# ishika28/Beyond-Binary-Fake-User-Detection-A-Credibility-Aware-Graph-based-Recommender-System

Hardware: NVIDIA B200
Metric: edges/sec (3-layer cred-weighted LightGCN fwd+bwd) (higher is better)
Workload: dtype f32

## Files before the change

### beyond-binary-fake-user-detection-a-credibility-aware-graph-based-recommender-system_b200/_lib.py

```python
from __future__ import annotations

import ctypes as C
import os
import pathlib
import subprocess

import torch

PKG_DIR = pathlib.Path(__file__).resolve().parent
LIB_PATH = PKG_DIR / "libcredgcn.so"
CSRC_DIR = PKG_DIR / "csrc"

VARIANTS = {"cu": 0, "v2": 1, "da": 2}
ORDERS = {"jacobi": 0, "gs": 1}
PRECISIONS = {"fp32": 0, "bf16x3": 1, "bf16": 2}
OPTIONS = {"L2_TABLE_BYTES": 0, "SPARSE_FIRST_ADJOINT": 1, "PDL": 2, "P2P_ONESHOT_MAX": 3, "P2P_TIMING": 4,
           "P2P_TIMEOUT_MS": 5, "EVAL_DEBUG": 6, "HOT_ROWS": 7, "EVAL_GROUPS": 8,
           "TOPK_CHUNK_USERS": 9}
LONG_ROW = 256
CHUNK = 256


class CgxError(RuntimeError):
    pass


class CsrStruct(C.Structure):
    _fields_ = [
        ("n_rows", C.c_int32), ("n_cols", C.c_int32), ("nnz", C.c_int64),
        ("indptr", C.c_void_p), ("idx", C.c_void_p), ("val_fwd", C.c_void_p), ("val_bwd", C.c_void_p),
        ("perm", C.c_void_p), ("n_long", C.c_int32), ("n_chunks", C.c_int32),
        ("chunk_ptr", C.c_void_p), ("chunk_row", C.c_void_p),
        ("n_huge", C.c_int32), ("reserved_", C.c_int32), ("arrive", C.c_void_p), ("work", C.c_void_p),
        ("idx_hint", C.c_void_p),
    ]


_P = C.c_void_p
_CSR = C.POINTER(CsrStruct)
_SIGNATURES = {
    "cgx_last_error": (C.c_char_p, []),
    "cgx_version": (C.c_int, []),
    "cgx_launch_count": (C.c_uint64, []),
    "cgx_emb_dim_supported": (C.c_int, [C.c_int32]),
    "cgx_set_option": (C.c_int, [C.c_int, C.c_int64, C.POINTER(C.c_int64)]),
    "cgx_get_option": (C.c_int64, [C.c_int]),
    "cgx_hot_hints_workspace_bytes": (C.c_size_t, [C.c_int32]),
    "cgx_hot_hints": (C.c_int, [_P, C.c_int64, C.c_int32, _P, C.c_int32, _P, _P, C.c_size_t, _P]),
    "cgx_comm_status": (C.c_int, [_P, C.c_size_t, C.c_int, C.POINTER(C.c_uint32)]),
    "cgx_graph_build_workspace_bytes": (C.c_size_t, [C.c_int64, C.c_int32, C.c_int32]),
    "cgx_graph_build": (C.c_int, [_P, _P, C.c_int64, C.c_int32, C.c_int32, _P, C.c_int, _P, _P, _P, _P, _P, _P,
                                  _P, _P, _P, _P, _P, _P, _P, _P, _P, C.c_int, _P, C.c_size_t, _P]),
    "cgx_user_csr": (C.c_int, [_P, _P, C.c_int64, C.c_int32, C.c_int32, _P, _P, _P, C.c_size_t, _P]),
    "cgx_row_schedule_workspace_bytes": (C.c_size_t, [C.c_int32]),
    "cgx_row_schedule": (C.c_int, [_P, C.c_int32, _P, C.POINTER(C.c_int32), C.POINTER(C.c_int32),
                                   C.POINTER(C.c_int32), _P, C.c_size_t, _P]),
    "cgx_row_schedule_chunks": (C.c_int, [C.c_int32, C.c_int32, C.c_int32, _P, _P, _P, C.c_size_t, _P]),
    "cgx_row_schedule_work": (C.c_int, [_P, _P, C.c_int32, C.c_int32, C.c_int32, _P, _P, _P, _P]),
    "cgx_spmm_workspace_bytes": (C.c_size_t, [_CSR, C.c_int32]),
    "cgx_spmm": (C.c_int, [_CSR, C.c_int, C.c_int32, _P, _P, _P, _P, C.c_float, _P, C.c_size_t, _P]),
    "cgx_spmm_sparse_rows": (C.c_int, [_CSR, C.c_int, C.c_int32, _P, _P, _P, _P, _P, C.c_float, _P, C.c_size_t, _P]),
    "cgx_row_flags": (C.c_int, [_P, C.c_int64, C.c_int32, _P, _P]),
    "cgx_spmm_ex": (C.c_int, [_CSR, C.c_int, C.c_int32, _P, _P, _P, _P, _P, _P, C.c_float, _P, C.c_size_t, _P]),
    "cgx_spmm_set_l2_table_bytes": (C.c_int64, [C.c_int64]),
    "cgx_propagate_workspace_bytes": (C.c_size_t, [_CSR, _CSR, C.c_int32]),
    "cgx_propagate_workspace_bytes_for": (C.c_size_t, [_CSR, _CSR, C.c_int32, C.c_int]),
    "cgx_propagate_fwd": (C.c_int, [_CSR, _CSR, C.c_int, C.c_int32, C.c_int32, _P, _P, _P, _P, _P,
                                    C.c_size_t, _P]),
    "cgx_propagate_fwd_layers": (C.c_int, [_CSR, _CSR, C.c_int, C.c_int32, C.c_int32, _P, _P, _P, _P, C.c_int32,
                                           C.c_int32, _P, _P, _P, _P, C.c_size_t, _P]),
    "cgx_propagate_bwd": (C.c_int, [_CSR, _CSR, C.c_int, C.c_int32, C.c_int32, _P, _P, _P, _P, _P,
                                    C.c_size_t, _P]),
    "cgx_propagate_bwd_flagged": (C.c_int, [_CSR, _CSR, C.c_int, C.c_int32, C.c_int32, _P, _P, _P, _P, _P, _P, _P,
                                            C.c_size_t, _P]),
    "cgx_propagate_bwd_frontier": (C.c_int, [_CSR, _CSR, C.c_int, C.c_int32, C.c_int32, _P, _P, _P, _P, _P, _P,
                                             _P, _P, C.c_size_t, _P]),
    "cgx_batch_frontier": (C.c_int, [_CSR, _P, _P, _P, C.c_int64, _P, _P, _P]),
    "cgx_bpr_mark_rows": (C.c_int, [_P, C.c_int64, C.c_int32, _P, _P, _P]),
    "cgx_bpr_clear_rows": (C.c_int, [_P, C.c_int64, C.c_int32, C.c_int32, _P, _P, _P, _P, _P]),
    "cgx_bpr_workspace_bytes": (C.c_size_t, [C.c_int64, C.c_int32, C.c_int32]),
    "cgx_bpr_plan_workspace_bytes": (C.c_size_t, [C.c_int64]),
    "cgx_bpr_plan": (C.c_int, [_P, _P, _P, C.c_int64, C.c_int32, C.c_int32, _P, _P, C.c_size_t, _P]),
    "cgx_bpr_fwd_bwd": (C.c_int, [_P, _P, _P, C.c_int64, C.c_int64, _P, C.c_int32, C.c_int32, C.c_int32, _P, _P, _P,
                                  _P, _P,
                                  C.c_float, C.c_float, _P, _P, _P, _P, _P, _P, C.c_size_t, _P]),
    "cgx_bpr_apply_ego": (C.c_int, [_P, _P, C.c_int64, C.c_int32, C.c_int32, _P, _P, _P, _P, _P]),
    "cgx_sampler_build_workspace_bytes": (C.c_size_t, [C.c_int32]),
    "cgx_sampler_build": (C.c_int, [_P, C.c_int32, C.c_double, _P, _P, _P, _P, _P, _P, C.c_size_t, _P]),
    "cgx_sample_triples": (C.c_int, [_P, C.c_int64, _P, _P, C.c_int32, _P, _P, _P, _P, _P, C.c_float,
                                     C.c_int32, C.c_uint64, C.c_uint64, _P, _P, _P, _P]),
    "cgx_tick": (C.c_int, [_P, _P]),
    "cgx_adam_step": (C.c_int, [_P, _P, _P, _P, C.c_int64, _P, _P, _P, _P, C.c_int64, C.c_float, C.c_float,
                                C.c_float, C.c_float, _P, C.c_int64, _P]),
    "cgx_comm_alloc": (C.c_int, [C.c_size_t, C.POINTER(C.c_void_p)]),
    "cgx_comm_free": (C.c_int, [_P]),
    "cgx_comm_ipc_handle": (C.c_int, [_P, _P]),
    "cgx_comm_ipc_open": (C.c_int, [_P, C.POINTER(C.c_void_p)]),
    "cgx_comm_ipc_close": (C.c_int, [_P]),
    "cgx_comm_allreduce": (C.c_int, [C.c_int, C.c_int, C.POINTER(C.c_void_p), C.c_size_t, C.c_size_t, C.c_size_t,
                                     C.c_int64, _P, _P]),
    "cgx_comm_allgather": (C.c_int, [C.c_int, C.c_int, C.POINTER(C.c_void_p), _P, C.c_size_t, C.c_size_t, C.c_int64,
                                     _P, _P]),
    "cgx_comm_allreduce_nvls": (C.c_int, [C.c_int, C.c_int, C.POINTER(C.c_void_p), _P, C.c_size_t, C.c_size_t,
                                          C.c_size_t, C.c_int64, _P, _P]),
    "cgx_comm_timing": (C.c_int, [_P]),
    "cgx_spmm_set_push_peers": (C.c_int, [C.POINTER(C.c_void_p), C.c_int]),
    "cgx_spmm_push": (C.c_int, [_CSR, C.c_int, C.c_int32, _P, _P, C.c_size_t, C.c_int, C.c_int, C.c_int32, _P,
                                C.c_size_t, _P]),
    "cgx_comm_allreduce_pushed": (C.c_int, [C.c_int, C.c_int, C.POINTER(C.c_void_p), C.c_size_t, C.c_size_t,
                                            C.c_size_t, C.c_int64, C.c_int32, C.c_int32, _P, _P]),
    "cgx_eval_topk_workspace_bytes": (C.c_size_t, [C.c_int64, C.c_int32, C.c_int32, C.c_int32, C.c_int]),
    "cgx_eval_topk": (C.c_int, [_P, C.c_int64, _P, _P, C.c_int32, C.c_int32, _P, _P, C.c_int32, C.c_int, _P,
                                _P, _P, C.c_size_t, _P]),
    "cgx_score_candidates": (C.c_int, [_P, _P, C.c_int64, C.c_int32, C.c_int32, _P, _P, _P, _P]),
    "cgx_eval_candidates": (C.c_int, [_P, C.c_int64, _P, _P, _P, _P, C.c_int32, C.c_int32, C.c_uint64, _P, _P]),
    "cgx_rank_candidates": (C.c_int, [_P, _P, C.c_int64, C.c_int32, _P, _P]),
    "cgx_eval_topk_uses_tensor_cores": (C.c_int, [C.c_int32, C.c_int32, C.c_int]),
    "cgx_eval_metrics_workspace_bytes": (C.c_size_t, [C.c_int64, C.c_int32]),
    "cgx_eval_metrics": (C.c_int, [_P, C.c_int64, C.c_int32, _P, _P, _P, _P, C.c_int32, _P, C.c_int32, _P, C.c_int64,
                                   _P, _P, _P, _P, C.c_size_t, _P]),
    "cgx_eval_coverage": (C.c_int, [_P, C.c_int32, C.c_int32, _P, _P]),
}
EXPORTED = tuple(_SIGNATURES)

_lib = None


def build_library(verbose: bool = False) -> pathlib.Path:
    out = subprocess.run(["make", "-C", str(CSRC_DIR), "-j8"], capture_output=True, text=True)
    if verbose or out.returncode != 0:
        print(out.stdout[-4000:], out.stderr[-4000:])
    if out.returncode != 0:
        raise CgxError("building libcredgcn.so failed (see output above)")
    return LIB_PATH


def lib() -> C.CDLL:
    global _lib
    if _lib is None:
        if not LIB_PATH.exists():
            raise CgxError(
                f"{LIB_PATH} is missing: the sm_100a extension has not been built. Run "
                f"`python -c 'import __graft_entry__ as g; g.build()'` (or `make -C {CSRC_DIR}`). "
                "There is no CPU fallback.")
        handle = C.CDLL(str(LIB_PATH))
        for name, (res, args) in _SIGNATURES.items():
            fn = getattr(handle, name)
            fn.restype, fn.argtypes = res, args
        _lib = handle
        for name, key in OPTIONS.items():
            env = os.environ.get(f"CGX_OPT_{name}")
            if env is not None:
                handle.cgx_set_option(key, int(env), None)
    return _lib


def set_option(name: str, value: int) -> int:
    prev = C.c_int64(0)
    check(lib().cgx_set_option(OPTIONS[name], int(value), C.byref(prev)))
    return int(prev.value)


def get_option(name: str) -> int:
    return int(lib().cgx_get_option(OPTIONS[name]))


def check(status: int) -> None:
    if status != 0:
        raise CgxError(f"libcredgcn error {status}: {lib().cgx_last_error().decode()}")


def ptr(t: torch.Tensor | None):
    if t is None:
        return None
    if not t.is_cuda:
        raise CgxError("credgcn ops need CUDA tensors: there is no CPU fallback")
    if not t.is_contiguous():
        raise CgxError("credgcn ops need contiguous tensors")
    return C.c_void_p(t.data_ptr())


def stream_ptr(device=None):
    return C.c_void_p(torch.cuda.current_stream(device).cuda_stream)


def workspace(nbytes: int, device) -> torch.Tensor:
    return torch.empty(max(int(nbytes), 256), dtype=torch.uint8, device=device)
```

### beyond-binary-fake-user-detection-a-credibility-aware-graph-based-recommender-system_b200/csrc/spmm.cu

```cuda
#include "common.cuh"

namespace cgx {

constexpr int SP_THREADS = 256;

__device__ __forceinline__ void fma4(float4& a, float v, const float4& x) {
  a.x = fmaf(v, x.x, a.x);
  a.y = fmaf(v, x.y, a.y);
  a.z = fmaf(v, x.z, a.z);
  a.w = fmaf(v, x.w, a.w);
}
__device__ __forceinline__ float4 add4(const float4& a, const float4& b) {
  return make_float4(a.x + b.x, a.y + b.y, a.z + b.z, a.w + b.w);
}
__device__ __forceinline__ float4 scale4(const float4& a, float s) {
  return make_float4(a.x * s, a.y * s, a.z * s, a.w * s);
}

enum { POL_NORMAL = 0, POL_FIRST = 1, POL_LAST = 2 };
template <int POL>
__device__ __forceinline__ void ld256(const float4* p, float4& a, float4& b) {
  if (POL == POL_LAST) {
    asm volatile("ld.global.nc.L1::no_allocate.L2::evict_last.v8.f32 {%0,%1,%2,%3,%4,%5,%6,%7}, [%8];"
                 : "=f"(a.x), "=f"(a.y), "=f"(a.z), "=f"(a.w), "=f"(b.x), "=f"(b.y), "=f"(b.z), "=f"(b.w)
                 : "l"(p));
  } else if (POL == POL_FIRST) {
    asm volatile("ld.global.nc.L1::no_allocate.L2::evict_first.v8.f32 {%0,%1,%2,%3,%4,%5,%6,%7}, [%8];"
                 : "=f"(a.x), "=f"(a.y), "=f"(a.z), "=f"(a.w), "=f"(b.x), "=f"(b.y), "=f"(b.z), "=f"(b.w)
                 : "l"(p));
  } else {
    asm volatile("ld.global.nc.v8.f32 {%0,%1,%2,%3,%4,%5,%6,%7}, [%8];"
                 : "=f"(a.x), "=f"(a.y), "=f"(a.z), "=f"(a.w), "=f"(b.x), "=f"(b.y), "=f"(b.z), "=f"(b.w)
                 : "l"(p));
  }
}
template <int POL>
__device__ __forceinline__ void ld256_rw(const float4* p, float4& a, float4& b) {
  if (POL == POL_FIRST) {
    asm volatile("ld.global.L1::no_allocate.L2::evict_first.v8.f32 {%0,%1,%2,%3,%4,%5,%6,%7}, [%8];"
                 : "=f"(a.x), "=f"(a.y), "=f"(a.z), "=f"(a.w), "=f"(b.x), "=f"(b.y), "=f"(b.z), "=f"(b.w)
                 : "l"(p)
                 : "memory");
  } else {
    asm volatile("ld.global.v8.f32 {%0,%1,%2,%3,%4,%5,%6,%7}, [%8];"
                 : "=f"(a.x), "=f"(a.y), "=f"(a.z), "=f"(a.w), "=f"(b.x), "=f"(b.y), "=f"(b.z), "=f"(b.w)
                 : "l"(p)
                 : "memory");
  }
}
template <int POL>
__device__ __forceinline__ void st256(float4* p, const float4& a, const float4& b) {
  if (POL == POL_FIRST) {
    asm volatile("st.global.L2::evict_first.v8.f32 [%0], {%1,%2,%3,%4,%5,%6,%7,%8};" ::"l"(p), "f"(a.x), "f"(a.y),
                 "f"(a.z), "f"(a.w), "f"(b.x), "f"(b.y), "f"(b.z), "f"(b.w)
                 : "memory");
  } else {
    asm volatile("st.global.v8.f32 [%0], {%1,%2,%3,%4,%5,%6,%7,%8};" ::"l"(p), "f"(a.x), "f"(a.y), "f"(a.z), "f"(a.w),
                 "f"(b.x), "f"(b.y), "f"(b.z), "f"(b.w)
                 : "memory");
  }
}
template <bool STREAM>
__device__ __forceinline__ int32_t ld_idx(const int32_t* p) {
  if (!STREAM) return __ldg(p);
  int32_t v;
  asm volatile("ld.global.nc.L1::no_allocate.b32 %0, [%1];" : "=r"(v) : "l"(p));
  return v;
}
template <bool STREAM>
__device__ __forceinline__ float ld_val(const float* p) {
  if (!STREAM) return __ldg(p);
  float v;
  asm volatile("ld.global.nc.L1::no_allocate.f32 %0, [%1];" : "=f"(v) : "l"(p));
  return v;
}

template <int G>
__device__ __forceinline__ unsigned group_mask() {
  if (G == 32) return 0xffffffffu;
  const unsigned lane = threadIdx.x & 31;
  return ((1u << (G & 31)) - 1u) << (lane & ~(G - 1));
}

template <int G, int V, bool HOT>
__device__ __forceinline__ void ld_row(const float4* __restrict__ X, int32_t c, int lane, float4 (&x)[V]) {
  constexpr int ROW4 = G * V;
  if constexpr (V == 2) {
    if constexpr (HOT) {
      const float4* p = X + int64_t(c & 0x7fffffff) * ROW4 + 2 * lane;
      if (c < 0) ld256<POL_LAST>(p, x[0], x[1]);
      else ld256<POL_FIRST>(p, x[0], x[1]);
    } else {
      ld256<POL_NORMAL>(X + int64_t(c) * ROW4 + 2 * lane, x[0], x[1]);
    }
  } else {
#pragma unroll
    for (int v = 0; v < V; ++v) x[v] = __ldg(X + int64_t(c) * ROW4 + lane * V + v);
  }
}

template <int G, int V, int UNR, bool NZ, bool HOT>
__device__ __forceinline__ void gather_batches(const int32_t* __restrict__ idx, const float* __restrict__ val,
                                               int32_t len, const float4* __restrict__ X, int lane,
                                               unsigned mask, int32_t c_nxt, float w_nxt, float4 (&acc)[V],
                                               const uint8_t* __restrict__ nz) {
  idx += G + lane;
  val += G + lane;
  for (int32_t rem = len; rem > 0; rem -= G, idx += G, val += G) {
    const int32_t c = c_nxt;
    float w = w_nxt;
    if (NZ) {
      if (w != 0.f && __ldg(nz + c) == 0) w = 0.f;
    }
    if (G + lane < rem) {
      c_nxt = ld_idx<HOT>(idx);
      w_nxt = ld_val<HOT>(val);
    }
    const int cnt = rem < G ? rem : G;
    for (int j0 = 0; j0 < cnt; j0 += UNR) {
      float4 x[UNR][V];
      float ww[UNR];
#pragma unroll
      for (int t = 0; t < UNR; ++t) {
        const int j = j0 + t;
        const int src = (j < G) ? j : (G - 1);
        const int32_t cj = __shfl_sync(mask, c, src, G);
        ww[t] = __shfl_sync(mask, w, src, G);
        if (j < cnt && (!NZ || ww[t] != 0.f)) {
          ld_row<G, V, HOT>(X, cj, lane, x[t]);
        } else {
          ww[t] = 0.f;
#pragma unroll
          for (int v = 0; v < V; ++v) x[t][v] = make_float4(0.f, 0.f, 0.f, 0.f);
        }
      }
#pragma unroll
      for (int t = 0; t < UNR; ++t) {
#pragma unroll
        for (int v = 0; v < V; ++v) fma4(acc[v], ww[t], x[t][v]);
      }
    }
  }
}

__constant__ char* c_push_base[16];
struct SpmmPush {
  unsigned long long off;
  int32_t rows_per;
  int32_t rank;
};

template <int G, int V, bool STREAM>
__device__ __forceinline__ void epilogue(int64_t row, int lane, const float4 (&y)[V], float4* __restrict__ Y,
                                         const float4* ACC_IN, float4* ACC_OUT, float acc_scale,
                                         const uint8_t* __restrict__ acc_nz, const SpmmPush ps) {
  constexpr int ROW4 = G * V;
  constexpr int POL = STREAM ? POL_FIRST : POL_NORMAL;
  const int64_t o = row * ROW4 + lane * V;
  float4 a[V];
#pragma unroll
  for (int v = 0; v < V; ++v) a[v] = make_float4(0.f, 0.f, 0.f, 0.f);
  if (ACC_OUT != nullptr && ACC_IN != nullptr && (acc_nz == nullptr || __ldg(acc_nz + row) != 0)) {
    if constexpr (V == 2) ld256_rw<POL>(ACC_IN + o, a[0], a[1]);
    else {
#pragma unroll
      for (int v = 0; v < V; ++v) a[v] = ACC_IN[o + v];
    }
  }
  if (ps.rows_per > 0) {
    const int owner = int(row / ps.rows_per);
    float4* ypush = reinterpret_cast<float4*>(c_push_base[owner] + ps.off) +
                    (int64_t(ps.rank) * ps.rows_per + (row - int64_t(owner) * ps.rows_per)) * ROW4 + lane * V;
    if constexpr (V == 2) st256<POL_NORMAL>(ypush, y[0], y[1]);
    else {
#pragma unroll
      for (int v = 0; v < V; ++v) ypush[v] = y[v];
    }
  }
  if (Y != nullptr) {
    if constexpr (V == 2) st256<POL>(Y + o, y[0], y[1]);
    else {
#pragma unroll
      for (int v = 0; v < V; ++v) Y[o + v] = y[v];
    }
  }
  if (ACC_OUT != nullptr) {
#pragma unroll
    for (int v = 0; v < V; ++v) a[v] = scale4(add4(a[v], y[v]), acc_scale);
    if constexpr (V == 2) st256<POL>(ACC_OUT + o, a[0], a[1]);
    else {
#pragma unroll
      for (int v = 0; v < V; ++v) ACC_OUT[o + v] = a[v];
    }
  }
}

struct SpmmSched {
  const int32_t* perm;
  const int32_t* chunk_ptr;
  int32_t* arrive;
  int32_t n_chunks, n_huge;
};

template <int G, int V, int UNR, int MINB, bool NZ, bool PUSH, bool HOT>
__global__ void __launch_bounds__(SP_THREADS, MINB) k_spmm(const int32_t* __restrict__ idx,
                                                           const float* __restrict__ val, int64_t n_items,
                                                           SpmmSched sc, const float4* __restrict__ X,
                                                           float4* __restrict__ Y, const float4* ACC_IN,
                                                           float4* ACC_OUT, float acc_scale, float4* partial,
                                                           const uint8_t* __restrict__ nz,
                                                           const uint8_t* __restrict__ acc_nz,
                                                           const uint8_t* __restrict__ out_rows,
                                                           const int4* __restrict__ work, const SpmmPush ps_in) {
  const SpmmPush ps = PUSH ? ps_in : SpmmPush{0ull, 0, 0};
  constexpr int ROW4 = G * V;
  asm volatile("griddepcontrol.launch_dependents;");
  const int lane = threadIdx.x & (G - 1);
  const uint32_t item = (blockIdx.x * uint32_t(SP_THREADS) + threadIdx.x) / G;
  const unsigned mask = group_mask<G>();
  float4 acc[V];
#pragma unroll
  for (int v = 0; v < V; ++v) acc[v] = make_float4(0.f, 0.f, 0.f, 0.f);
  if (item >= n_items) return;
  const int4 wd = __ldg(work + item);
  const int64_t begin = (int64_t(wd.y) << 32) | uint32_t(wd.x);
  idx += begin;
  val += begin;
  int32_t cf = 0;
  float wf = 0.f;
  if (lane < wd.z) {
    cf = ld_idx<HOT>(idx + lane);
    wf = ld_val<HOT>(val + lane);
  }
  asm volatile("griddepcontrol.wait;" ::: "memory");
  if (NZ && !PUSH && out_rows != nullptr &&
      __ldg(out_rows + (item >= sc.n_chunks ? wd.w : __ldg(sc.perm + wd.w))) == 0)
    return;
  gather_batches<G, V, UNR, NZ, HOT>(idx, val, wd.z, X, lane, mask, cf, wf, acc, nz);
  if (item >= sc.n_chunks) {
    epilogue<G, V, HOT>(wd.w, lane, acc, Y, ACC_IN, ACC_OUT, acc_scale, acc_nz, ps);
    return;
  }
  const int32_t k = wd.w;
#pragma unroll
  for (int v = 0; v < V; ++v) __stcg(partial + int64_t(item) * ROW4 + lane * V + v, acc[v]);
  if (k < sc.n_huge) return;
  const int32_t c0 = __ldg(sc.chunk_ptr + k), c1 = __ldg(sc.chunk_ptr + k + 1);
  __threadfence();
  __syncwarp(mask);
  int prev = 0;
  if (lane == 0) prev = atomicAdd(sc.arrive + k, 1);
  prev = __shfl_sync(mask, prev, 0, G);
  if (prev != c1 - c0 - 1) return;
  __threadfence();
#pragma unroll
  for (int v = 0; v < V; ++v) acc[v] = make_float4(0.f, 0.f, 0.f, 0.f);
  for (int c = c0; c < c1; ++c) {
#pragma unroll
    for (int v = 0; v < V; ++v) acc[v] = add4(acc[v], __ldcg(partial + int64_t(c) * ROW4 + lane * V + v));
  }
  epilogue<G, V, HOT>(int64_t(__ldg(sc.perm + k)), lane, acc, Y, ACC_IN, ACC_OUT, acc_scale, acc_nz, ps);
  if (lane == 0) sc.arrive[k] = 0;
}

template <int G, int V>
__global__ void __launch_bounds__(SP_THREADS) k_spmm_finish(SpmmSched sc, const float4* __restrict__ partial,
                                                            float4* __restrict__ Y, const float4* ACC_IN,
                                                            float4* ACC_OUT, float acc_scale,
                                                            const uint8_t* __restrict__ acc_nz,
                                                            const uint8_t* __restrict__ out_rows, const SpmmPush ps) {
  constexpr int GROUPS = SP_THREADS / G;
  constexpr int ROW4 = G * V;
  __shared__ float4 red[GROUPS][ROW4];
  const int k = blockIdx.x;
  if (out_rows != nullptr && __ldg(out_rows + __ldg(sc.perm + k)) == 0) return;
  const int lane = threadIdx.x & (G - 1), grp = threadIdx.x / G;
  const int c0 = __ldg(sc.chunk_ptr + k), c1 = __ldg(sc.chunk_ptr + k + 1);
  float4 acc[V];
#pragma unroll
  for (int v = 0; v < V; ++v) acc[v] = make_float4(0.f, 0.f, 0.f, 0.f);
  for (int c = c0 + grp; c < c1; c += GROUPS) {
#pragma unroll
    for (int v = 0; v < V; ++v) acc[v] = add4(acc[v], __ldg(partial + int64_t(c) * ROW4 + lane * V + v));
  }
#pragma unroll
  for (int v = 0; v < V; ++v) red[grp][lane * V + v] = acc[v];
  __syncthreads();
  if (grp == 0) {
#pragma unroll
    for (int v = 0; v < V; ++v) {
      float4 s = red[0][lane * V + v];
      for (int g = 1; g < GROUPS; ++g) s = add4(s, red[g][lane * V + v]);
      acc[v] = s;
    }
    epilogue<G, V, false>(int64_t(__ldg(sc.perm + k)), lane, acc, Y, ACC_IN, ACC_OUT, acc_scale, acc_nz, ps);
  }
}

__global__ void k_scale(const float4* __restrict__ in, float4* __restrict__ out, int64_t n4, float s) {
  int64_t p = int64_t(blockIdx.x) * blockDim.x + threadIdx.x;
  if (p < n4) out[p] = scale4(in[p], s);
}

__global__ void k_row_flags(const uint4* __restrict__ X, int64_t n4, int32_t row4, uint8_t* __restrict__ flags) {
  const int64_t p = int64_t(blockIdx.x) * blockDim.x + threadIdx.x;
  if (p >= n4) return;
  const uint4 v = X[p];
  if ((v.x | v.y | v.z | v.w) & 0x7fffffffu) flags[p / row4] = 1;
}

static int row_flags(const float* X, int64_t n_rows, int32_t d, uint8_t* flags, cudaStream_t stream) {
  CGX_CUDA(cudaMemsetAsync(flags, 0, size_t(n_rows), stream));
  const int64_t n4 = n_rows * d / 4;
  if (n4 == 0) return CGX_OK;
  k_row_flags<<<(unsigned)ceil_div(n4, 256), 256, 0, stream>>>(reinterpret_cast<const uint4*>(X), n4, d / 4, flags);
  CGX_LAUNCH_CHECK();
  return CGX_OK;
}

template <int G, int V, int UNR, int MINB, bool NZ, bool PUSH, bool HOT>
static int launch_spmm(const cgx_csr* m, const float* val, const float* X, float* Y, const float* ACC_IN,
                       float* ACC_OUT, float acc_scale, void* workspace, size_t workspace_bytes,
                       cudaStream_t stream, const uint8_t* nz, const uint8_t* acc_nz, const uint8_t* out_rows,
                       const SpmmPush ps) {
  constexpr int GROUPS = SP_THREADS / G;
  float4* partial = nullptr;
  if (m->n_long > 0) {
    size_t need = size_t(m->n_chunks) * G * V * sizeof(float4);
    CGX_REQUIRE(workspace != nullptr && workspace_bytes >= need, CGX_ERR_WORKSPACE,
                "spmm: workspace too small for %d long-row chunks", m->n_chunks);
    partial = static_cast<float4*>(workspace);
  }
  SpmmSched sc{m->perm, m->chunk_ptr, m->arrive, m->n_chunks, m->n_huge};
  const int64_t items = int64_t(m->n_chunks) + (m->n_rows - m->n_long);
  cudaLaunchConfig_t cfg = {};
  cfg.gridDim = dim3((unsigned)ceil_div(items, GROUPS));
  cfg.blockDim = dim3(SP_THREADS);
  cfg.dynamicSmemBytes = 0;
  cfg.stream = stream;
  cudaLaunchAttribute attr[1];
  attr[0].id = cudaLaunchAttributeProgrammaticStreamSerialization;
  attr[0].val.programmaticStreamSerializationAllowed = option(CGX_OPT_PDL) != 0 ? 1 : 0;
  cfg.attrs = attr;
  cfg.numAttrs = 1;
  CGX_CUDA(cudaLaunchKernelEx(&cfg, k_spmm<G, V, UNR, MINB, NZ, PUSH, HOT>, HOT ? m->idx_hint : m->idx, val, items, sc,
                              reinterpret_cast<const float4*>(X), reinterpret_cast<float4*>(Y),
                              reinterpret_cast<const float4*>(ACC_IN), reinterpret_cast<float4*>(ACC_OUT), acc_scale,
                              partial, nz, acc_nz, out_rows, static_cast<const int4*>(m->work), ps));
  CGX_LAUNCH_CHECK();
  if (m->n_huge > 0) {
    k_spmm_finish<G, V><<<(unsigned)m->n_huge, SP_THREADS, 0, stream>>>(
        sc, partial, reinterpret_cast<float4*>(Y), reinterpret_cast<const float4*>(ACC_IN),
        reinterpret_cast<float4*>(ACC_OUT), acc_scale, acc_nz, out_rows, ps);
    CGX_LAUNCH_CHECK();
  }
  return CGX_OK;
}

#define CGX_SPMM_ARGS m, val, X, Y, ACC_IN, ACC_OUT, acc_scale, ws, ws_bytes, stream, nz, acc_nz, out_rows, ps

template <int G, int V, int UNR>
static int spmm_flavour(const cgx_csr* m, const float* val, const float* X, float* Y, const float* ACC_IN,
                        float* ACC_OUT, float acc_scale, void* ws, size_t ws_bytes, cudaStream_t stream,
                        const uint8_t* nz, const uint8_t* acc_nz, const uint8_t* out_rows, const SpmmPush ps,
                        bool hot) {
  const bool push = ps.rows_per > 0;
  if constexpr (V == 2) {
    if (hot && nz == nullptr) {
      if (push) return launch_spmm<G, V, UNR, 4, false, true, true>(CGX_SPMM_ARGS);
      return launch_spmm<G, V, UNR, 4, false, false, true>(CGX_SPMM_ARGS);
    }
  }
  if (push) {
    if (nz) return launch_spmm<G, V, UNR, 4, true, true, false>(CGX_SPMM_ARGS);
    return launch_spmm<G, V, UNR, 4, false, true, false>(CGX_SPMM_ARGS);
  }
  if (nz) return launch_spmm<G, V, UNR, 4, true, false, false>(CGX_SPMM_ARGS);
  return launch_spmm<G, V, UNR, 4, false, false, false>(CGX_SPMM_ARGS);
}

#define CGX_FLAVOUR_ARGS m, val, X, Y, ACC_IN, ACC_OUT, acc_scale, ws, ws_bytes, stream, nz, acc_nz, out_rows, ps, hot

static int spmm_dispatch(const cgx_csr* m, int use_bwd, int32_t d, const float* X, float* Y, const float* ACC_IN,
                         float* ACC_OUT, float acc_scale, void* ws, size_t ws_bytes, cudaStream_t stream,
                         const uint8_t* nz = nullptr, const SpmmPush ps = SpmmPush{0ull, 0, 0},
                         const uint8_t* acc_nz = nullptr, const uint8_t* out_rows = nullptr) {
  CGX_REQUIRE(m && m->perm && m->work && (m->nnz == 0 || (m->idx && m->val_fwd && m->val_bwd)) && X, CGX_ERR_ARG,
              "spmm: NULL pointer (cgx_csr needs idx, both value arrays and the cgx_row_schedule* outputs)");
  CGX_REQUIRE(m->n_long == 0 || (m->chunk_ptr && m->arrive), CGX_ERR_ARG, "spmm: chunk tables missing");
  CGX_REQUIRE(Y || ACC_OUT || ps.rows_per > 0, CGX_ERR_ARG, "spmm: no output requested");
  CGX_REQUIRE(out_rows == nullptr || (nz != nullptr && ps.rows_per == 0), CGX_ERR_ARG,
              "spmm: an output-row mask needs gather flags and no push mode");
  const float* val = use_bwd ? m->val_bwd : m->val_fwd;
  if (m->n_rows == 0) return CGX_OK;
  const bool beyond_l2 = int64_t(m->n_cols) * int64_t(d) * 4 > option(CGX_OPT_L2_TABLE_BYTES);
  const bool hot = beyond_l2 && m->idx_hint != nullptr && option(CGX_OPT_HOT_ROWS) != 0;
  switch (d) {
    case 16: return spmm_flavour<4, 1, 4>(CGX_FLAVOUR_ARGS);
    case 32: return spmm_flavour<8, 1, 8>(CGX_FLAVOUR_ARGS);
    case 64:
      if (beyond_l2) return spmm_flavour<8, 2, 4>(CGX_FLAVOUR_ARGS);
      return spmm_flavour<16, 1, 8>(CGX_FLAVOUR_ARGS);
    case 128:
      if (beyond_l2) return spmm_flavour<16, 2, 4>(CGX_FLAVOUR_ARGS);
      return spmm_flavour<32, 1, 8>(CGX_FLAVOUR_ARGS);
    case 256: return spmm_flavour<32, 2, 4>(CGX_FLAVOUR_ARGS);
    default:
      set_error("spmm: emb_dim %d unsupported (16, 32, 64, 128, 256)", d);
      return CGX_ERR_UNSUPPORTED;
  }
}

__global__ void k_hot_flags(const int32_t* __restrict__ col_by_degree, int32_t n_hot, uint8_t* __restrict__ hot) {
  const int32_t k = blockIdx.x * blockDim.x + threadIdx.x;
  if (k < n_hot) hot[__ldg(col_by_degree + k)] = 1;
}
__global__ void k_hot_hint(const int32_t* __restrict__ idx, int64_t nnz, const uint8_t* __restrict__ hot,
                           int32_t* __restrict__ out) {
  const int64_t p = int64_t(blockIdx.x) * blockDim.x + threadIdx.x;
  if (p >= nnz) return;
  const int32_t c = idx[p];
  out[p] = __ldg(hot + c) ? (c | int32_t(0x80000000u)) : c;
}

static size_t spmm_ws(const cgx_csr* m, int32_t d) { return align_up(size_t(m ? m->n_chunks : 0) * d * 4); }

}

using namespace cgx;

extern "C" size_t cgx_spmm_workspace_bytes(const cgx_csr* m, int32_t d) { return spmm_ws(m, d); }

extern "C" int cgx_spmm(const cgx_csr* m, int use_bwd_values, int32_t d, const float* X, float* Y,
                        const float* ACC_IN, float* ACC_OUT, float acc_scale, void* workspace,
                        size_t workspace_bytes, void* stream) {
  return spmm_dispatch(m, use_bwd_values, d, X, Y, ACC_IN, ACC_OUT, acc_scale, workspace, workspace_bytes,
                       static_cast<cudaStream_t>(stream));
}

extern "C" int cgx_spmm_sparse_rows(const cgx_csr* m, int use_bwd_values, int32_t d, const float* X,
                                    const uint8_t* x_row_nonzero, float* Y, const float* ACC_IN, float* ACC_OUT,
                                    float acc_scale, void* workspace, size_t workspace_bytes, void* stream) {
  CGX_REQUIRE(x_row_nonzero != nullptr, CGX_ERR_ARG, "spmm_sparse_rows: NULL flags");
  return spmm_dispatch(m, use_bwd_values, d, X, Y, ACC_IN, ACC_OUT, acc_scale, workspace, workspace_bytes,
                       static_cast<cudaStream_t>(stream), x_row_nonzero);
}

extern "C" int cgx_spmm_ex(const cgx_csr* m, int use_bwd_values, int32_t d, const float* X, const uint8_t* x_row_nonzero,
                           float* Y, const float* ACC_IN, const uint8_t* acc_row_nonzero, float* ACC_OUT,
                           float acc_scale, void* workspace, size_t workspace_bytes, void* stream) {
  return spmm_dispatch(m, use_bwd_values, d, X, Y, ACC_IN, ACC_OUT, acc_scale, workspace, workspace_bytes,
                       static_cast<cudaStream_t>(stream), x_row_nonzero, SpmmPush{0ull, 0, 0}, acc_row_nonzero);
}

extern "C" int64_t cgx_spmm_set_l2_table_bytes(int64_t bytes) {
  int64_t old = 0;
  cgx_set_option(CGX_OPT_L2_TABLE_BYTES, bytes, &old);
  return old;
}

extern "C" size_t cgx_hot_hints_workspace_bytes(int32_t n_cols) { return align_up(size_t(n_cols > 0 ? n_cols : 0)) + 256; }

extern "C" int cgx_hot_hints(const int32_t* idx, int64_t nnz, int32_t n_cols, const int32_t* col_by_degree,
                             int32_t n_hot, int32_t* idx_hint, void* workspace, size_t workspace_bytes,
                             void* stream_) {
  cudaStream_t stream = static_cast<cudaStream_t>(stream_);
  CGX_REQUIRE(nnz >= 0 && n_cols > 0 && col_by_degree && idx_hint && (nnz == 0 || idx) && n_hot >= 0 &&
                  n_hot <= n_cols,
              CGX_ERR_ARG, "hot_hints: bad argument");
  CGX_REQUIRE(workspace != nullptr && workspace_bytes >= cgx_hot_hints_workspace_bytes(n_cols), CGX_ERR_WORKSPACE,
              "hot_hints: workspace too small");
  uint8_t* hot = static_cast<uint8_t*>(workspace);
  CGX_CUDA(cudaMemsetAsync(hot, 0, size_t(n_cols), stream));
  if (n_hot > 0) {
    k_hot_flags<<<(unsigned)ceil_div(n_hot, 256), 256, 0, stream>>>(col_by_degree, n_hot, hot);
    CGX_LAUNCH_CHECK();
  }
  if (nnz > 0) {
    k_hot_hint<<<(unsigned)ceil_div(nnz, 256), 256, 0, stream>>>(idx, nnz, hot, idx_hint);
    CGX_LAUNCH_CHECK();
  }
  return CGX_OK;
}

extern "C" int cgx_spmm_set_push_peers(void* const* peer_bases, int world) {
  CGX_REQUIRE(peer_bases != nullptr && world >= 1 && world <= 16, CGX_ERR_ARG, "spmm_set_push_peers: bad argument");
  char* h[16] = {nullptr};
  for (int p = 0; p < world; ++p) h[p] = static_cast<char*>(peer_bases[p]);
  CGX_CUDA(cudaMemcpyToSymbol(c_push_base, h, sizeof(h)));
  return CGX_OK;
}

extern "C" int cgx_spmm_push(const cgx_csr* m, int use_bwd_values, int32_t d, const float* X,
                             const uint8_t* x_row_nonzero, size_t stage_off, int rank, int world, int32_t rows_per,
                             void* workspace, size_t workspace_bytes, void* stream) {
  CGX_REQUIRE(m != nullptr && world >= 1 && world <= 16 && rank >= 0 && rank < world && rows_per > 0 &&
                  int64_t(rows_per) * world >= m->n_rows && stage_off % 16 == 0,
              CGX_ERR_ARG, "spmm_push: bad rank / world / rows_per");
  const SpmmPush ps{(unsigned long long)stage_off, rows_per, rank};
  return spmm_dispatch(m, use_bwd_values, d, X, nullptr, nullptr, nullptr, 1.0f, workspace, workspace_bytes,
                       static_cast<cudaStream_t>(stream), x_row_nonzero, ps);
}

extern "C" int cgx_row_flags(const float* X, int64_t n_rows, int32_t d, uint8_t* flags, void* stream) {
  CGX_REQUIRE(X && flags && n_rows >= 0 && d > 0 && d % 4 == 0, CGX_ERR_ARG, "row_flags: bad argument");
  return row_flags(X, n_rows, d, flags, static_cast<cudaStream_t>(stream));
}

__device__ __forceinline__ int64_t clamp_row(int64_t x, int64_t n) { return (x < 0 || x >= n) ? 0 : x; }
__global__ void k_batch_frontier(const int64_t* __restrict__ indptr, const int32_t* __restrict__ idx,
                                 const int64_t* __restrict__ users, const int64_t* __restrict__ pos,
                                 const int64_t* __restrict__ neg, int64_t B, int32_t U, int32_t I,
                                 uint8_t* __restrict__ flags, uint8_t* __restrict__ flags_u) {
  const int64_t t = (int64_t(blockIdx.x) * blockDim.x + threadIdx.x) / 32;
  const int lane = threadIdx.x & 31;
  if (t >= B) return;
  const int64_t u = clamp_row(users[t], U);
  if (lane == 0) {
    flags[clamp_row(pos[t], I)] = 1;
    flags[clamp_row(neg[t], I)] = 1;
    if (flags_u != nullptr) flags_u[u] = 1;
  }
  const int64_t end = indptr[u + 1];
  for (int64_t j = indptr[u] + lane; j < end; j += 32) flags[idx[j]] = 1;
}

extern "C" int cgx_batch_frontier(const cgx_csr* by_user, const int64_t* users, const int64_t* pos,
                                  const int64_t* neg, int64_t B, uint8_t* flags_i, uint8_t* flags_u,
                                  void* stream_) {
  cudaStream_t stream = static_cast<cudaStream_t>(stream_);
  CGX_REQUIRE(by_user && by_user->indptr && (by_user->nnz == 0 || by_user->idx) && users && pos && neg && flags_i,
              CGX_ERR_ARG, "batch_frontier: NULL pointer");
  CGX_REQUIRE(B > 0 && B < (int64_t(1) << 29) && by_user->n_rows > 0 && by_user->n_cols > 0, CGX_ERR_ARG,
              "batch_frontier: bad batch size %lld or empty graph", (long long)B);
  CGX_CUDA(cudaMemsetAsync(flags_i, 0, size_t(by_user->n_cols), stream));
  if (flags_u != nullptr) CGX_CUDA(cudaMemsetAsync(flags_u, 0, size_t(by_user->n_rows), stream));
  k_batch_frontier<<<(unsigned)ceil_div(B * 32, 256), 256, 0, stream>>>(
      by_user->indptr, by_user->idx, users, pos, neg, B, by_user->n_rows, by_user->n_cols, flags_i, flags_u);
  CGX_LAUNCH_CHECK();
  return CGX_OK;
}

static size_t propagate_ws(const cgx_csr* by_user, const cgx_csr* by_item, int32_t d, int n_buf) {
  if (!by_user || !by_item) return 0;
  size_t long_ws = spmm_ws(by_user, d) > spmm_ws(by_item, d) ? spmm_ws(by_user, d) : spmm_ws(by_item, d);
  return n_buf * (align_up(size_t(by_user->n_rows) * d * 4) + align_up(size_t(by_item->n_rows) * d * 4)) + long_ws +
         align_up(size_t(by_user->n_rows)) + align_up(size_t(by_item->n_rows)) + 256;
}

extern "C" size_t cgx_propagate_workspace_bytes(const cgx_csr* by_user, const cgx_csr* by_item, int32_t d) {
  return propagate_ws(by_user, by_item, d, 2);
}

extern "C" size_t cgx_propagate_workspace_bytes_for(const cgx_csr* by_user, const cgx_csr* by_item, int32_t d,
                                                    int order) {
  return propagate_ws(by_user, by_item, d, order == CGX_ORDER_GS ? 1 : 2);
}

extern "C" int cgx_propagate_fwd(const cgx_csr* by_user, const cgx_csr* by_item, int order, int32_t K, int32_t d,
                                 const float* e0_u, const float* e0_i, float* out_u, float* out_i,
                                 void* workspace, size_t workspace_bytes, void* stream) {
  return cgx_propagate_fwd_layers(by_user, by_item, order, K, d, e0_u, e0_i, out_u, out_i, 0, K, nullptr, nullptr,
                                  nullptr, workspace, workspace_bytes, stream);
}

extern "C" int cgx_propagate_fwd_layers(const cgx_csr* by_user, const cgx_csr* by_item, int order, int32_t K,
                                        int32_t d, const float* e0_u, const float* e0_i, float* out_u, float* out_i,
                                        int32_t layer_begin, int32_t layer_end, const uint8_t* rows_u,
                                        const uint8_t* rows_i, const uint8_t* all_rows, void* workspace,
                                        size_t workspace_bytes, void* stream_) {
  cudaStream_t stream = static_cast<cudaStream_t>(stream_);
  CGX_REQUIRE(by_user && by_item && e0_u && e0_i && out_u && out_i, CGX_ERR_ARG, "propagate_fwd: NULL pointer");
  CGX_REQUIRE(K >= 1, CGX_ERR_ARG, "propagate_fwd: num_layers must be >= 1");
  CGX_REQUIRE(0 <= layer_begin && layer_begin <= layer_end && layer_end <= K, CGX_ERR_ARG,
              "propagate_fwd: layers [%d, %d) outside [0, %d)", layer_begin, layer_end, K);
  CGX_REQUIRE((rows_u == nullptr && rows_i == nullptr) || all_rows != nullptr, CGX_ERR_ARG,
              "propagate_fwd: output-row masks need all_rows");
  CGX_REQUIRE(order == CGX_ORDER_JACOBI || order == CGX_ORDER_GS, CGX_ERR_ARG, "propagate_fwd: bad order");
  CGX_REQUIRE(by_user->n_rows == by_item->n_cols && by_user->n_cols == by_item->n_rows, CGX_ERR_ARG,
              "propagate_fwd: operator shapes disagree");
  CGX_REQUIRE(workspace_bytes >= cgx_propagate_workspace_bytes_for(by_user, by_item, d, order), CGX_ERR_WORKSPACE,
              "propagate_fwd: workspace too small");
  const int64_t U = by_user->n_rows, I = by_item->n_rows;
  Arena ws(workspace, workspace_bytes);
  const bool one = order == CGX_ORDER_GS;
  float* ub[2];
  float* ib[2];
  ub[0] = ws.take<float>(U * d);
  ub[1] = one ? ub[0] : ws.take<float>(U * d);
  ib[0] = ws.take<float>(I * d);
  ib[1] = one ? ib[0] : ws.take<float>(I * d);
  size_t lws = spmm_ws(by_user, d) > spmm_ws(by_item, d) ? spmm_ws(by_user, d) : spmm_ws(by_item, d);
  void* lw = ws.take<char>(lws);
  CGX_REQUIRE(ws.ok, CGX_ERR_WORKSPACE, "propagate_fwd: workspace too small");
  const float s = 1.0f / float(K + 1);
  const SpmmPush nops{0ull, 0, 0};
  for (int k = layer_begin; k < layer_end; ++k) {
    const bool first = k == 0, last = k == K - 1;
    const float* cu = first ? e0_u : ub[(k - 1) & 1];
    const float* ci = first ? e0_i : ib[(k - 1) & 1];
    float* nu = ub[k & 1];
    float* ni = ib[k & 1];
    const float sc = last ? s : 1.0f;
    const uint8_t* mu = last ? rows_u : nullptr;
    const uint8_t* mi = last ? rows_i : nullptr;
    const bool need_ni = !last || order == CGX_ORDER_GS;
    CGX_TRY(spmm_dispatch(by_item, 0, d, cu, need_ni ? ni : nullptr, first ? e0_i : out_i, out_i, sc, lw, lws,
                          stream, mi ? all_rows : nullptr, nops, nullptr, mi));
    const float* src = order == CGX_ORDER_JACOBI ? ci : ni;
    CGX_TRY(spmm_dispatch(by_user, 0, d, src, last ? nullptr : nu, first ? e0_u : out_u, out_u, sc, lw, lws,
                          stream, mu ? all_rows : nullptr, nops, nullptr, mu));
  }
  return CGX_OK;
}

__global__ void k_scale_rows(const float4* __restrict__ in, const uint8_t* __restrict__ nz, float4* __restrict__ out,
                             int64_t n_rows, int32_t row4, float s) {
  const int64_t r = (int64_t(blockIdx.x) * blockDim.x + threadIdx.x) / 32;
  if (r >= n_rows || __ldg(nz + r) == 0) return;
  for (int p = threadIdx.x & 31; p < row4; p += 32) out[r * row4 + p] = scale4(in[r * row4 + p], s);
}

extern "C" int cgx_propagate_bwd(const cgx_csr* by_user, const cgx_csr* by_item, int order, int32_t K, int32_t d,
                                 const float* g_u, const float* g_i, float* d_e0_u, float* d_e0_i,
                                 void* workspace, size_t workspace_bytes, void* stream_) {
  return cgx_propagate_bwd_flagged(by_user, by_item, order, K, d, g_u, g_i, nullptr, nullptr, d_e0_u, d_e0_i, workspace,
                                   workspace_bytes, stream_);
}

extern "C" int cgx_propagate_bwd_flagged(const cgx_csr* by_user, const cgx_csr* by_item, int order, int32_t K,
                                         int32_t d, const float* g_u, const float* g_i, const uint8_t* g_u_rows,
                                         const uint8_t* g_i_rows, float* d_e0_u, float* d_e0_i, void* workspace,
                                         size_t workspace_bytes, void* stream_) {
  return cgx_propagate_bwd_frontier(by_user, by_item, order, K, d, g_u, g_i, g_u_rows, g_i_rows, nullptr, d_e0_u,
                                    d_e0_i, workspace, workspace_bytes, stream_);
}

extern "C" int cgx_propagate_bwd_frontier(const cgx_csr* by_user, const cgx_csr* by_item, int order, int32_t K,
                                          int32_t d, const float* g_u, const float* g_i, const uint8_t* g_u_rows,
                                          const uint8_t* g_i_rows, const uint8_t* front_i, float* d_e0_u,
                                          float* d_e0_i, void* workspace, size_t workspace_bytes, void* stream_) {
  cudaStream_t stream = static_cast<cudaStream_t>(stream_);
  CGX_REQUIRE((g_u_rows == nullptr) == (g_i_rows == nullptr), CGX_ERR_ARG,
              "propagate_bwd_flagged: pass both row-flag arrays or neither");
  CGX_REQUIRE(by_user && by_item && g_u && g_i && d_e0_u && d_e0_i, CGX_ERR_ARG, "propagate_bwd: NULL pointer");
  CGX_REQUIRE(K >= 1, CGX_ERR_ARG, "propagate_bwd: num_layers must be >= 1");
  CGX_REQUIRE(order == CGX_ORDER_JACOBI || order == CGX_ORDER_GS, CGX_ERR_ARG, "propagate_bwd: bad order");
  CGX_REQUIRE(workspace_bytes >= cgx_propagate_workspace_bytes_for(by_user, by_item, d, order), CGX_ERR_WORKSPACE,
              "propagate_bwd: workspace too small");
  const int64_t U = by_user->n_rows, I = by_item->n_rows;
  Arena ws(workspace, workspace_bytes);
  const bool one = order == CGX_ORDER_GS;
  float* ub[2];
  float* ib[2];
  ub[0] = ws.take<float>(U * d);
  ub[1] = one ? ub[0] : ws.take<float>(U * d);
  ib[0] = ws.take<float>(I * d);
  ib[1] = one ? ib[0] : ws.take<float>(I * d);
  size_t lws = spmm_ws(by_user, d) > spmm_ws(by_item, d) ? spmm_ws(by_user, d) : spmm_ws(by_item, d);
  void* lw = ws.take<char>(lws);
  CGX_REQUIRE(ws.ok, CGX_ERR_WORKSPACE, "propagate_bwd: workspace too small");
  const float s = 1.0f / float(K + 1);
  const bool given = g_u_rows != nullptr;
  const bool sparse = given || option(CGX_OPT_SPARSE_FIRST_ADJOINT) != 0;
  uint8_t* nz_u = given ? const_cast<uint8_t*>(g_u_rows) : ws.take<uint8_t>(U);
  uint8_t* nz_i = given ? const_cast<uint8_t*>(g_i_rows) : ws.take<uint8_t>(I);
  CGX_REQUIRE(ws.ok, CGX_ERR_WORKSPACE, "propagate_bwd: workspace too small");
  const uint8_t* front = sparse ? front_i : nullptr;
  if (order == CGX_ORDER_JACOBI) {
    const float* bu = g_u;
    const float* bi = g_i;
    if (sparse && !given) {
      CGX_TRY(row_flags(g_u, U, d, nz_u, stream));
      CGX_TRY(row_flags(g_i, I, d, nz_i, stream));
    }
    for (int k = 0; k < K; ++k) {
      const bool last = k == K - 1;
      float* nu = last ? d_e0_u : ub[k & 1];
      float* ni = last ? d_e0_i : ib[k & 1];
      const float sc = last ? s : 1.0f;
      const bool sp = sparse && k == 0;
      const SpmmPush nops{0ull, 0, 0};
      const uint8_t* bi_nz = sp ? nz_i : (k == 1 ? front : nullptr);
      CGX_TRY(spmm_dispatch(by_user, 1, d, bi, nullptr, g_u, nu, sc, lw, lws, stream, bi_nz, nops,
                            sparse ? nz_u : nullptr));
      CGX_TRY(spmm_dispatch(by_item, 1, d, bu, nullptr, g_i, ni, sc, lw, lws, stream, sp ? nz_u : nullptr, nops,
                            sparse ? nz_i : nullptr, k == 0 && !last ? front : nullptr));
      bu = nu;
      bi = ni;
    }
  } else {
    const float* bu = g_u;
    if (sparse && !given) {
      CGX_TRY(row_flags(g_u, U, d, nz_u, stream));
      CGX_TRY(row_flags(g_i, I, d, nz_i, stream));
    }
    const SpmmPush nops{0ull, 0, 0};
    for (int k = 0; k < K; ++k) {
      const bool last = k == K - 1;
      float* ni = ib[0];
      float* nu = last ? d_e0_u : ub[k & 1];
      const uint8_t* f0 = k == 0 ? front : nullptr;
      CGX_TRY(spmm_dispatch(by_item, 1, d, bu, nullptr, g_i, ni, 1.0f, lw, lws, stream,
                            sparse && k == 0 ? nz_u : nullptr, nops, sparse ? nz_i : nullptr, f0));
      CGX_TRY(spmm_dispatch(by_user, 1, d, ni, nullptr, g_u, nu, last ? s : 1.0f, lw, lws, stream, f0, nops,
                            sparse ? nz_u : nullptr));
      bu = nu;
    }
    const int64_t n4 = I * d / 4;
    if (given) {
      CGX_CUDA(cudaMemsetAsync(d_e0_i, 0, size_t(I) * d * 4, stream));
      if (I > 0) {
        k_scale_rows<<<(unsigned)ceil_div(I * 32, 256), 256, 0, stream>>>(
            reinterpret_cast<const float4*>(g_i), nz_i, reinterpret_cast<float4*>(d_e0_i), I, d / 4, s);
        CGX_LAUNCH_CHECK();
      }
    } else {
      k_scale<<<(unsigned)ceil_div(n4, 256), 256, 0, stream>>>(reinterpret_cast<const float4*>(g_i),
                                                               reinterpret_cast<float4*>(d_e0_i), n4, s);
      CGX_LAUNCH_CHECK();
    }
  }
  return CGX_OK;
}
```

### beyond-binary-fake-user-detection-a-credibility-aware-graph-based-recommender-system_b200/model.py

```python
from __future__ import annotations

import torch

from . import _lib
from ._lib import check, lib, ptr, stream_ptr, workspace
from .graph import CredGraph, graph_of


def _f32c(t: torch.Tensor) -> torch.Tensor:
    if t.dtype != torch.float32:
        raise _lib.CgxError(f"credgcn kernels are fp32, got {t.dtype}")
    return t.contiguous()


def _i64c(t, device) -> torch.Tensor:
    return torch.as_tensor(t, device=device).to(torch.int64).contiguous()


def propagate_forward(graph: CredGraph, e0_u, e0_i, num_layers: int, order: str):
    e0_u, e0_i = _f32c(e0_u), _f32c(e0_i)
    d = e0_u.shape[1]
    out_u, out_i = torch.empty_like(e0_u), torch.empty_like(e0_i)
    ws = graph.propagate_workspace(d, order)
    with torch.cuda.device(graph.device):
        check(lib().cgx_propagate_fwd(graph.by_user.ref(), graph.by_item.ref(), _lib.ORDERS[order], num_layers, d,
                                      ptr(e0_u), ptr(e0_i), ptr(out_u), ptr(out_i), ptr(ws), ws.numel(),
                                      stream_ptr(graph.device)))
    return out_u, out_i


def propagate_backward(graph: CredGraph, g_u, g_i, num_layers: int, order: str):
    g_u, g_i = _f32c(g_u), _f32c(g_i)
    d = g_u.shape[1]
    d_u, d_i = torch.empty_like(g_u), torch.empty_like(g_i)
    ws = graph.propagate_workspace(d, order)
    with torch.cuda.device(graph.device):
        check(lib().cgx_propagate_bwd(graph.by_user.ref(), graph.by_item.ref(), _lib.ORDERS[order], num_layers, d,
                                      ptr(g_u), ptr(g_i), ptr(d_u), ptr(d_i), ptr(ws), ws.numel(),
                                      stream_ptr(graph.device)))
    return d_u, d_i


def spmm(csr, x, use_bwd_values=False):
    x = _f32c(x)
    d = x.shape[1]
    y = torch.empty(csr.n_rows, d, dtype=torch.float32, device=x.device)
    ws = workspace(lib().cgx_spmm_workspace_bytes(csr.ref(), d), x.device)
    with torch.cuda.device(x.device):
        check(lib().cgx_spmm(csr.ref(), int(use_bwd_values), d, ptr(x), ptr(y), None, None, 1.0, ptr(ws),
                             ws.numel(), stream_ptr(x.device)))
    return y


def row_flags(x):
    x = _f32c(x)
    flags = torch.empty(x.shape[0], dtype=torch.uint8, device=x.device)
    with torch.cuda.device(x.device):
        check(lib().cgx_row_flags(ptr(x), x.shape[0], x.shape[1], ptr(flags), stream_ptr(x.device)))
    return flags


def spmm_sparse_rows(csr, x, flags=None, use_bwd_values=False):
    x = _f32c(x)
    flags = row_flags(x) if flags is None else flags
    d = x.shape[1]
    y = torch.empty(csr.n_rows, d, dtype=torch.float32, device=x.device)
    ws = workspace(lib().cgx_spmm_workspace_bytes(csr.ref(), d), x.device)
    with torch.cuda.device(x.device):
        check(lib().cgx_spmm_sparse_rows(csr.ref(), int(use_bwd_values), d, ptr(x), ptr(flags), ptr(y), None, None,
                                         1.0, ptr(ws), ws.numel(), stream_ptr(x.device)))
    return y


def bpr_plan(graph: CredGraph, users, pos, neg, plan=None):
    dev = graph.device
    users, pos, neg = _i64c(users, dev), _i64c(pos, dev), _i64c(neg, dev)
    B = users.numel()
    if plan is None:
        plan = torch.empty(3 * B, dtype=torch.int64, device=dev)
    ws = workspace(lib().cgx_bpr_plan_workspace_bytes(B), dev)
    with torch.cuda.device(dev):
        check(lib().cgx_bpr_plan(ptr(users), ptr(pos), ptr(neg), B, graph.num_users, graph.num_items, ptr(plan),
                                 ptr(ws), ws.numel(), stream_ptr(dev)))
    return plan


def batch_frontier(graph: CredGraph, users, pos, neg, flags=None, flags_u=None):
    dev = graph.device
    users, pos, neg = _i64c(users, dev), _i64c(pos, dev), _i64c(neg, dev)
    if flags is None:
        flags = torch.empty(graph.num_items, dtype=torch.uint8, device=dev)
    with torch.cuda.device(dev):
        check(lib().cgx_batch_frontier(graph.by_user.ref(), ptr(users), ptr(pos), ptr(neg), users.numel(), ptr(flags),
                                       ptr(flags_u), stream_ptr(dev)))
    return flags


def bpr_fused(graph: CredGraph, f_u, f_i, e0_u, e0_i, users, pos, neg, reg_weight, fair_weight=0.0, pop=None,
              g_u=None, g_i=None, plan=None, bufs=None, batch_total=0):
    dev = f_u.device
    f_u, f_i, e0_u, e0_i = _f32c(f_u), _f32c(f_i), _f32c(e0_u), _f32c(e0_i)
    users, pos, neg = _i64c(users, dev), _i64c(pos, dev), _i64c(neg, dev)
    B, d = users.numel(), f_u.shape[1]
    if plan is None:
        plan = bpr_plan(graph, users, pos, neg)
    if g_u is None:
        g_u = torch.zeros_like(f_u)
    if g_i is None:
        g_i = torch.zeros_like(f_i)
    if bufs is None:
        bufs = bpr_buffers(graph, B, dev)
    loss, ego_rows, ego_coef, ws = bufs
    pop_t = None if pop is None else _f32c(torch.as_tensor(pop, device=dev))
    with torch.cuda.device(dev):
        check(lib().cgx_bpr_fwd_bwd(ptr(users), ptr(pos), ptr(neg), B, int(batch_total), ptr(plan), graph.num_users,
                                    graph.num_items,
                                    d, ptr(f_u), ptr(f_i), ptr(e0_u), ptr(e0_i), ptr(pop_t), float(reg_weight),
                                    float(fair_weight), ptr(loss), ptr(g_u), ptr(g_i), ptr(ego_rows),
                                    ptr(ego_coef), ptr(ws), ws.numel(), stream_ptr(dev)))
    return loss, g_u, g_i, ego_rows, ego_coef


def bpr_buffers(graph: CredGraph, B: int, dev):
    return (torch.empty(1, dtype=torch.float32, device=dev), torch.empty(3 * B, dtype=torch.int32, device=dev),
            torch.empty(3 * B, dtype=torch.float32, device=dev),
            workspace(lib().cgx_bpr_workspace_bytes(B, graph.num_users, graph.num_items), dev))


def apply_ego(graph: CredGraph, ego_rows, ego_coef, e0_u, e0_i, d_e0_u, d_e0_i):
    with torch.cuda.device(e0_u.device):
        check(lib().cgx_bpr_apply_ego(ptr(ego_rows), ptr(ego_coef), ego_rows.numel(), graph.num_users,
                                      e0_u.shape[1], ptr(_f32c(e0_u)), ptr(_f32c(e0_i)), ptr(d_e0_u), ptr(d_e0_i),
                                      stream_ptr(e0_u.device)))


class _Propagate(torch.autograd.Function):

    @staticmethod
    def forward(ctx, e0_u, e0_i, graph, num_layers, order):
        ctx.graph, ctx.num_layers, ctx.order = graph, num_layers, order
        return propagate_forward(graph, e0_u.detach(), e0_i.detach(), num_layers, order)

    @staticmethod
    def backward(ctx, g_u, g_i):
        d_u, d_i = propagate_backward(ctx.graph, g_u, g_i, ctx.num_layers, ctx.order)
        return d_u, d_i, None, None, None


class _SpMM(torch.autograd.Function):

    @staticmethod
    def forward(ctx, x, graph, which):
        ctx.graph, ctx.which = graph, which
        return spmm(graph.by_user if which == "A" else graph.by_item, x.detach(), False)

    @staticmethod
    def backward(ctx, gy):
        csr = ctx.graph.by_item if ctx.which == "A" else ctx.graph.by_user
        return spmm(csr, gy, True), None, None


class _BprLoss(torch.autograd.Function):
    @staticmethod
    def forward(ctx, f_u, f_i, e0_u, e0_i, graph, users, pos, neg, reg_weight, fair_weight, pop):
        loss, g_u, g_i, ego_rows, ego_coef = bpr_fused(graph, f_u.detach(), f_i.detach(), e0_u.detach(),
                                                        e0_i.detach(), users, pos, neg, reg_weight, fair_weight, pop)
        ctx.graph = graph
        ctx.save_for_backward(g_u, g_i, ego_rows, ego_coef, e0_u.detach(), e0_i.detach())
        return loss.reshape(())

    @staticmethod
    def backward(ctx, g):
        g_u, g_i, ego_rows, ego_coef, e0_u, e0_i = ctx.saved_tensors
        d_e0_u, d_e0_i = torch.zeros_like(e0_u), torch.zeros_like(e0_i)
        apply_ego(ctx.graph, ego_rows, ego_coef, e0_u, e0_i, d_e0_u, d_e0_i)
        return g_u * g, g_i * g, d_e0_u * g, d_e0_i * g, None, None, None, None, None, None, None


def fused_bpr_loss(graph, f_u, f_i, e0_u, e0_i, users, pos, neg, reg_weight, fair_weight=0.0, pop=None):
    return _BprLoss.apply(f_u, f_i, e0_u, e0_i, graph, users, pos, neg, reg_weight, fair_weight, pop)


class _Base(torch.nn.Module):
    ORDER = "gs"

    def __init__(self, num_users, num_items, emb_dim, num_layers, M_ui, M_iu):
        super().__init__()
        self.num_users, self.num_items, self.num_layers = num_users, num_items, num_layers
        self.M_ui, self.M_iu = M_ui, M_iu
        self.graph = graph_of(M_ui, M_iu)
        if (self.graph.num_users, self.graph.num_items) != (num_users, num_items):
            raise ValueError("operator shapes do not match num_users / num_items")
        if not lib().cgx_emb_dim_supported(emb_dim):
            raise _lib.CgxError(f"emb_dim={emb_dim} unsupported: use 16, 32, 64, 128 or 256")
        self.user_emb = torch.nn.Embedding(num_users, emb_dim)
        self.item_emb = torch.nn.Embedding(num_items, emb_dim)
        torch.nn.init.xavier_uniform_(self.user_emb.weight)
        torch.nn.init.xavier_uniform_(self.item_emb.weight)

    def ego_tables(self):
        eu, ei = self.user_emb.weight, self.item_emb.weight
        eu.grad, ei.grad = torch.empty_like(eu), torch.empty_like(ei)
        return eu.data, ei.data, eu.grad, ei.grad

    def _final(self):
        return _Propagate.apply(self.user_emb.weight, self.item_emb.weight, self.graph, self.num_layers, self.ORDER)

    def _layers(self):
        u, i = self.user_emb.weight, self.item_emb.weight
        us, is_ = [u], [i]
        for _ in range(self.num_layers):
            i_new = _SpMM.apply(u, self.graph, "C")
            u_new = _SpMM.apply(i if self.ORDER == "jacobi" else i_new, self.graph, "A")
            u, i = u_new, i_new
            us.append(u)
            is_.append(i)
        return us, is_


class CredLightGCN(_Base):
    ORDER = "jacobi"

    def propagate_all_layers(self):
        return self._layers()

    def final_embeddings(self):
        return self._final()

    def score(self, users, items, e_u, e_i):
        return (e_u[users] * e_i[items]).sum(dim=1)

    def l2_reg(self, users, pos_items, neg_items):
        eu, ep, en = self.user_emb.weight[users], self.item_emb.weight[pos_items], self.item_emb.weight[neg_items]
        return (eu.norm(2, dim=1).pow(2) + ep.norm(2, dim=1).pow(2) + en.norm(2, dim=1).pow(2)).mean()

    def fused_loss(self, users, pos_items, neg_items, e_u, e_i, lambda_reg, lambda_fair=0.0, pop=None):
        return fused_bpr_loss(self.graph, e_u, e_i, self.user_emb.weight, self.item_emb.weight, users, pos_items,
                              neg_items, lambda_reg, lambda_fair, pop)


class LightGCN(_Base):
    ORDER = "gs"

    def propagate(self):
        return self._final()

    def get_user_item_emb(self):
        return self.propagate()

    def bpr_loss(self, users, pos_items, neg_items, user_emb, item_emb, reg_weight: float):
        return fused_bpr_loss(self.graph, user_emb, item_emb, self.user_emb.weight, self.item_emb.weight, users,
                              pos_items, neg_items, reg_weight)


class RawLightGCN(torch.nn.Module):
    ORDER = "jacobi"

    def __init__(self, num_users, num_items, emb_dim, num_layers, norm_adj):
        super().__init__()
        from .graph import NormAdj
        if not isinstance(norm_adj, NormAdj):
            raise TypeError("expected the handle returned by credgcn.graph.build_norm_adj")
        self.num_users, self.num_items, self.num_layers = num_users, num_items, num_layers
        self.num_nodes = num_users + num_items
        self.norm_adj, self.graph = norm_adj, norm_adj.graph
        if not lib().cgx_emb_dim_supported(emb_dim):
            raise _lib.CgxError(f"emb_dim={emb_dim} unsupported: use 16, 32, 64, 128 or 256")
        self.emb = torch.nn.Embedding(self.num_nodes, emb_dim)
        torch.nn.init.xavier_uniform_(self.emb.weight)

    def ego_tables(self):
        w, U = self.emb.weight, self.num_users
        w.grad = torch.empty_like(w)
        return w.data[:U], w.data[U:], w.grad[:U], w.grad[U:]

    def propagate(self):
        w = self.emb.weight
        fu, fi = _Propagate.apply(w[: self.num_users], w[self.num_users:], self.graph, self.num_layers, self.ORDER)
        return torch.cat([fu, fi], dim=0)

    def get_user_item_emb(self):
        x = self.propagate()
        return x[: self.num_users], x[self.num_users:]

    def bpr_loss(self, users, pos_items, neg_items, user_emb, item_emb, reg_weight: float):
        w = self.emb.weight
        return fused_bpr_loss(self.graph, user_emb, item_emb, w[: self.num_users], w[self.num_users:], users,
                              pos_items, neg_items, reg_weight)


class FusedAdam:

    def __init__(self, user_weight: torch.Tensor, item_weight: torch.Tensor, lr=1e-3, betas=(0.9, 0.999), eps=1e-8,
                 grads=None):
        self.params = (user_weight, item_weight)
        self.grads = grads
        self.lr, self.betas, self.eps = float(lr), (float(betas[0]), float(betas[1])), float(eps)
        self.m = [torch.zeros_like(p) for p in self.params]
        self.v = [torch.zeros_like(p) for p in self.params]
        self.step_dev = torch.zeros(1, dtype=torch.int64, device=user_weight.device)

    def _grads(self):
        return self.grads if self.grads is not None else tuple(p.grad for p in self.params)

    def zero_grad(self, set_to_none: bool = False):
        for g in self._grads():
            if g is not None:
                g.zero_()

    @torch.no_grad()
    def step(self):
        pu, pi = self.params
        gu, gi = self._grads()
        dev = pu.device
        with torch.cuda.device(dev):
            st = stream_ptr(dev)
            check(lib().cgx_tick(ptr(self.step_dev), st))
            check(lib().cgx_adam_step(ptr(pu.data), ptr(_f32c(gu)), ptr(self.m[0]), ptr(self.v[0]), pu.numel(),
                                      ptr(pi.data), ptr(_f32c(gi)), ptr(self.m[1]), ptr(self.v[1]), pi.numel(),
                                      self.lr, self.betas[0], self.betas[1], self.eps, ptr(self.step_dev), 0, st))

    def state_dict(self):
        return {"step": int(self.step_dev.item()), "exp_avg": self.m, "exp_avg_sq": self.v, "lr": self.lr,
                "betas": self.betas, "eps": self.eps}


class TrainStep:

    DEFER_HEADROOM = 2 << 30

    def __init__(self, model: _Base | RawLightGCN, lr=1e-3, reg_weight=1e-4, fair_weight=0.0, pop=None, optimizer=None,
                 sampler=None):
        self.model, self.graph = model, model.graph
        self.reg, self.fair = float(reg_weight), float(fair_weight)
        self._eu, self._ei, self._gu, self._gi = model.ego_tables()
        eu, ei = self._eu, self._ei
        dev = eu.device
        self.pop = None if pop is None else torch.as_tensor(pop, dtype=torch.float32, device=dev).contiguous()
        self._f_u, self._f_i = torch.empty_like(eu), torch.empty_like(ei)
        self.g_u, self.g_i = torch.zeros_like(eu), torch.zeros_like(ei)
        self.nz_u = torch.zeros(eu.shape[0], dtype=torch.uint8, device=dev)
        self.nz_i = torch.zeros(ei.shape[0], dtype=torch.uint8, device=dev)
        self.front_i = torch.zeros(ei.shape[0], dtype=torch.uint8, device=dev)
        self.batch_u = torch.zeros(eu.shape[0], dtype=torch.uint8, device=dev)
        self.opt = optimizer or FusedAdam(eu, ei, lr=lr, grads=(self._gu, self._gi))
        self.sampler = sampler
        self.phase_events = None
        self.side = torch.cuda.Stream(device=dev)
        self.tick = torch.zeros(1, dtype=torch.int64, device=dev)
        self._bufs = {}
        self._graph = None
        self._defer_final = None
        self._fws = self._all_rows = None
        self._pending = False
        self._final_error = None

    @property
    def f_u(self) -> torch.Tensor:
        self._complete_final()
        return self._f_u

    @property
    def f_i(self) -> torch.Tensor:
        self._complete_final()
        return self._f_i

    def _defers_final(self, d, order, beyond_l2):
        if self.model.num_layers < 2 or not beyond_l2:
            return False
        g = self.graph
        need = lib().cgx_propagate_workspace_bytes_for(g.by_user.ref(), g.by_item.ref(), d, order)
        free, _ = torch.cuda.mem_get_info(g.device)
        return free >= need + self.DEFER_HEADROOM

    @torch.no_grad()
    def _complete_final(self):
        if self._final_error is not None:
            raise self._final_error
        if not self._pending:
            return
        m, g = self.model, self.graph
        eu, ei = self._eu, self._ei
        d, K, order = eu.shape[1], m.num_layers, _lib.ORDERS[m.ORDER]
        dev = eu.device
        with torch.cuda.device(dev):
            rest_u = torch.eq(self.batch_u, 0).view(torch.uint8)
            rest_i = torch.eq(self.front_i, 0).view(torch.uint8)
            try:
                check(lib().cgx_propagate_fwd_layers(g.by_user.ref(), g.by_item.ref(), order, K, d, ptr(eu), ptr(ei),
                                                     ptr(self._f_u), ptr(self._f_i), K - 1, K, ptr(rest_u),
                                                     ptr(rest_i), ptr(self._all_rows), ptr(self._fws),
                                                     self._fws.numel(), stream_ptr(dev)))
            except _lib.CgxError as e:
                self._final_error = e
                raise
        self._pending = False

    def _mark(self, marks):
        if self.phase_events is not None:
            ev = torch.cuda.Event(enable_timing=True)
            ev.record(torch.cuda.current_stream(self.graph.device))
            marks.append(ev)

    def _batch_bufs(self, B, dev):
        if B not in self._bufs:
            self._bufs[B] = (torch.empty(3 * B, dtype=torch.int64, device=dev), bpr_buffers(self.graph, B, dev))
        return self._bufs[B]

    @torch.no_grad()
    def forward_backward(self, users, pos, neg):
        m, g = self.model, self.graph
        eu, ei = self._eu, self._ei
        d, K, order = eu.shape[1], m.num_layers, _lib.ORDERS[m.ORDER]
        ws = g.propagate_workspace(d, order)
        dev = eu.device
        users, pos, neg = _i64c(users, dev), _i64c(pos, dev), _i64c(neg, dev)
        plan, bufs = self._batch_bufs(users.numel(), dev)
        beyond_l2 = g.num_items * d * 4 > _lib.get_option("L2_TABLE_BYTES")
        if self._defer_final is None:
            self._defer_final = self._defers_final(d, order, beyond_l2)
        defer = bool(self._defer_final) and K >= 2
        if defer and self._fws is None:
            self._fws = workspace(lib().cgx_propagate_workspace_bytes_for(g.by_user.ref(), g.by_item.ref(), d, order),
                                  dev)
            self._all_rows = torch.ones(max(g.num_users, g.num_items), dtype=torch.uint8, device=dev)
        front = self.front_i if beyond_l2 or defer else None
        marks = []
        self._pending, self._final_error = False, None
        with torch.cuda.device(dev):
            main = torch.cuda.current_stream(dev)
            self._mark(marks)
            self.side.wait_stream(main)
            with torch.cuda.stream(self.side):
                bpr_plan(g, users, pos, neg, plan)
                if front is not None:
                    batch_frontier(g, users, pos, neg, front, self.batch_u if defer else None)
            st = stream_ptr(dev)
            if defer:
                fws = self._fws
                check(lib().cgx_propagate_fwd_layers(g.by_user.ref(), g.by_item.ref(), order, K, d, ptr(eu), ptr(ei),
                                                     ptr(self._f_u), ptr(self._f_i), 0, K - 1, None, None, None,
                                                     ptr(fws), fws.numel(), st))
                main.wait_stream(self.side)
                check(lib().cgx_propagate_fwd_layers(g.by_user.ref(), g.by_item.ref(), order, K, d, ptr(eu), ptr(ei),
                                                     ptr(self._f_u), ptr(self._f_i), K - 1, K, ptr(self.batch_u),
                                                     ptr(self.front_i), ptr(self._all_rows), ptr(fws), fws.numel(),
                                                     st))
                self._mark(marks)
                self._pending = True
            else:
                check(lib().cgx_propagate_fwd(g.by_user.ref(), g.by_item.ref(), order, K, d, ptr(eu), ptr(ei),
                                              ptr(self._f_u), ptr(self._f_i), ptr(ws), ws.numel(), st))
                self._mark(marks)
                main.wait_stream(self.side)
            loss, _, _, ego_rows, ego_coef = bpr_fused(g, self._f_u, self._f_i, eu, ei, users, pos, neg, self.reg,
                                                       self.fair, self.pop, self.g_u, self.g_i, plan, bufs)
            n_ent = ego_rows.numel()
            check(lib().cgx_bpr_mark_rows(ptr(ego_rows), n_ent, g.num_users, ptr(self.nz_u), ptr(self.nz_i), st))
            self._mark(marks)
            check(lib().cgx_propagate_bwd_frontier(g.by_user.ref(), g.by_item.ref(), order, K, d, ptr(self.g_u),
                                                   ptr(self.g_i), ptr(self.nz_u), ptr(self.nz_i), ptr(front),
                                                   ptr(self._gu), ptr(self._gi), ptr(ws), ws.numel(), st))
            self._mark(marks)
            apply_ego(g, ego_rows, ego_coef, eu, ei, self._gu, self._gi)
            check(lib().cgx_bpr_clear_rows(ptr(ego_rows), n_ent, g.num_users, d, ptr(self.g_u), ptr(self.g_i),
                                           ptr(self.nz_u), ptr(self.nz_i), st))
        if self.phase_events is not None:
            self.phase_events.append(marks)
        return loss

    def __call__(self, users, pos, neg):
        loss = self.forward_backward(users, pos, neg)
        self.opt.step()
        return loss

    @torch.no_grad()
    def _sampled_step(self, users):
        dev = self.graph.device
        with torch.cuda.device(dev):
            check(lib().cgx_tick(ptr(self.tick), stream_ptr(dev)))
        pos, neg = self.sampler.sample(users, offset=0, offset_dev=self.tick)
        return self.__call__(users, pos, neg)

    def capture(self, batch: int, preserve_state: bool = True):
        if self.sampler is None:
            raise _lib.CgxError("TrainStep.capture needs a TripleSampler (pass sampler=...)")
        dev = self.graph.device
        self._g_users = torch.zeros(batch, dtype=torch.int64, device=dev)
        keep = self.phase_events
        self.phase_events = None
        warm = torch.cuda.Stream(device=dev)
        warm.wait_stream(torch.cuda.current_stream(dev))
        with torch.cuda.stream(warm):
            state = opt_state = None
            if preserve_state:
                state = [self._eu.clone(), self._ei.clone()]
                opt_state = ([t.clone() for t in self.opt.m], [t.clone() for t in self.opt.v],
                             self.opt.step_dev.clone(), self.tick.clone()) if isinstance(self.opt, FusedAdam) else None
            for _ in range(2):
                self._sampled_step(self._g_users)
            if state is not None:
                self._eu.copy_(state[0])
                self._ei.copy_(state[1])
            if opt_state is not None:
                for dst, src in zip(self.opt.m, opt_state[0]):
                    dst.copy_(src)
                for dst, src in zip(self.opt.v, opt_state[1]):
                    dst.copy_(src)
                self.opt.step_dev.copy_(opt_state[2])
                self.tick.copy_(opt_state[3])
        torch.cuda.current_stream(dev).wait_stream(warm)
        torch.cuda.synchronize(dev)
        self._graph = torch.cuda.CUDAGraph()
        with torch.cuda.graph(self._graph):
            self._g_loss = self._sampled_step(self._g_users)
        self._g_pending = self._pending
        self.phase_events = keep
        return self

    def step(self, users):
        if self.sampler is None:
            raise _lib.CgxError("TrainStep.step needs a TripleSampler (pass sampler=...)")
        if self._graph is not None and users.numel() == self._g_users.numel() and self.phase_events is None:
            self._g_users.copy_(users, non_blocking=True)
            self._graph.replay()
            self._pending, self._final_error = self._g_pending, None
            return self._g_loss
        return self._sampled_step(_i64c(users, self.graph.device))
```

### include/credgcn.h

```cpp
#ifndef CREDGCN_H_
#define CREDGCN_H_

#include <stddef.h>
#include <stdint.h>

#if defined(__GNUC__)
#pragma GCC visibility push(default)
#endif

#ifdef __cplusplus
extern "C" {
#endif

typedef enum {
  CGX_OK = 0,
  CGX_ERR_ARG = -1,
  CGX_ERR_WORKSPACE = -2,
  CGX_ERR_CUDA = -3,
  CGX_ERR_UNSUPPORTED = -4
} cgx_status;

typedef enum { CGX_VARIANT_CU = 0, CGX_VARIANT_V2 = 1, CGX_VARIANT_DA = 2 } cgx_variant;
typedef enum { CGX_ORDER_JACOBI = 0, CGX_ORDER_GS = 1 } cgx_order;
typedef enum { CGX_SCORE_FP32 = 0, CGX_SCORE_BF16X3 = 1, CGX_SCORE_BF16 = 2 } cgx_score_precision;

const char* cgx_last_error(void);
int cgx_version(void);
uint64_t cgx_launch_count(void);
int cgx_emb_dim_supported(int32_t d);

typedef enum {
  CGX_OPT_L2_TABLE_BYTES = 0,
  CGX_OPT_SPARSE_FIRST_ADJOINT = 1,
  CGX_OPT_PDL = 2,
  CGX_OPT_P2P_ONESHOT_MAX = 3,
  CGX_OPT_P2P_TIMING = 4,
  CGX_OPT_P2P_TIMEOUT_MS = 5,
  CGX_OPT_EVAL_DEBUG = 6,
  CGX_OPT_HOT_ROWS = 7,
  CGX_OPT_EVAL_GROUPS = 8,
  CGX_OPT_TOPK_CHUNK_USERS = 9,
  CGX_OPT_COUNT_ = 10
} cgx_option;
int cgx_set_option(int option, int64_t value, int64_t* previous);
int64_t cgx_get_option(int option);


typedef struct {
  int32_t n_rows;
  int32_t n_cols;
  int64_t nnz;
  const int64_t* indptr;
  const int32_t* idx;
  const float* val_fwd;
  const float* val_bwd;
  const int32_t* perm;
  int32_t n_long;
  int32_t n_chunks;
  const int32_t* chunk_ptr;
  const int32_t* chunk_row;
  int32_t n_huge;
  int32_t reserved_;
  int32_t* arrive;
  const void* work;
  const int32_t* idx_hint;
} cgx_csr;

#define CGX_LONG_ROW 256
#define CGX_CHUNK 256
#define CGX_HUGE_ROW 16384

size_t cgx_graph_build_workspace_bytes(int64_t num_edges, int32_t num_users, int32_t num_items);

int cgx_graph_build(const int32_t* edges_u, const int32_t* edges_i, int64_t num_edges,
                    int32_t num_users, int32_t num_items, const float* cred, int variant,
                    const float* alpha, const int32_t* deg_i_weights, int32_t* deg_u, int32_t* deg_i,
                    int64_t* samp_indptr, int32_t* samp_idx,
                    int64_t* user_indptr, int32_t* user_idx, float* user_val_fwd, float* user_val_bwd,
                    int64_t* item_indptr, int32_t* item_idx, float* item_val_fwd, float* item_val_bwd,
                    int64_t* nnz_out, int deg_only, void* workspace, size_t workspace_bytes, void* stream);

int cgx_user_csr(const int32_t* edges_u, const int32_t* edges_i, int64_t num_edges, int32_t num_users,
                 int32_t num_items, int64_t* indptr, int32_t* idx, void* workspace,
                 size_t workspace_bytes, void* stream);

size_t cgx_row_schedule_workspace_bytes(int32_t n_rows);
int cgx_row_schedule(const int64_t* indptr, int32_t n_rows, int32_t* perm, int32_t* n_long_host,
                     int32_t* n_chunks_host, int32_t* n_huge_host, void* workspace, size_t workspace_bytes,
                     void* stream);
int cgx_row_schedule_chunks(int32_t n_rows, int32_t n_long, int32_t n_chunks, int32_t* chunk_ptr,
                            int32_t* chunk_row, void* workspace, size_t workspace_bytes, void* stream);
int cgx_row_schedule_work(const int64_t* indptr, const int32_t* perm, int32_t n_rows, int32_t n_long,
                          int32_t n_chunks, const int32_t* chunk_ptr, const int32_t* chunk_row, void* work,
                          void* stream);

size_t cgx_hot_hints_workspace_bytes(int32_t n_cols);
int cgx_hot_hints(const int32_t* idx, int64_t nnz, int32_t n_cols, const int32_t* col_by_degree, int32_t n_hot,
                  int32_t* idx_hint, void* workspace, size_t workspace_bytes, void* stream);


size_t cgx_spmm_workspace_bytes(const cgx_csr* m, int32_t d);
int cgx_spmm(const cgx_csr* m, int use_bwd_values, int32_t d, const float* X, float* Y,
             const float* ACC_IN, float* ACC_OUT, float acc_scale,
             void* workspace, size_t workspace_bytes, void* stream);

int cgx_spmm_sparse_rows(const cgx_csr* m, int use_bwd_values, int32_t d, const float* X,
                         const uint8_t* x_row_nonzero, float* Y, const float* ACC_IN, float* ACC_OUT,
                         float acc_scale, void* workspace, size_t workspace_bytes, void* stream);
int cgx_row_flags(const float* X, int64_t n_rows, int32_t d, uint8_t* flags, void* stream);
int cgx_spmm_ex(const cgx_csr* m, int use_bwd_values, int32_t d, const float* X, const uint8_t* x_row_nonzero,
                float* Y, const float* ACC_IN, const uint8_t* acc_row_nonzero, float* ACC_OUT, float acc_scale,
                void* workspace, size_t workspace_bytes, void* stream);

int64_t cgx_spmm_set_l2_table_bytes(int64_t bytes);

size_t cgx_propagate_workspace_bytes(const cgx_csr* by_user, const cgx_csr* by_item, int32_t d);
size_t cgx_propagate_workspace_bytes_for(const cgx_csr* by_user, const cgx_csr* by_item, int32_t d, int order);

int cgx_propagate_fwd(const cgx_csr* by_user, const cgx_csr* by_item, int order, int32_t num_layers,
                      int32_t d, const float* e0_u, const float* e0_i, float* out_u, float* out_i,
                      void* workspace, size_t workspace_bytes, void* stream);
int cgx_propagate_fwd_layers(const cgx_csr* by_user, const cgx_csr* by_item, int order, int32_t num_layers,
                             int32_t d, const float* e0_u, const float* e0_i, float* out_u, float* out_i,
                             int32_t layer_begin, int32_t layer_end, const uint8_t* rows_u, const uint8_t* rows_i,
                             const uint8_t* all_rows, void* workspace, size_t workspace_bytes, void* stream);

int cgx_propagate_bwd(const cgx_csr* by_user, const cgx_csr* by_item, int order, int32_t num_layers,
                      int32_t d, const float* g_u, const float* g_i, float* d_e0_u, float* d_e0_i,
                      void* workspace, size_t workspace_bytes, void* stream);
int cgx_propagate_bwd_flagged(const cgx_csr* by_user, const cgx_csr* by_item, int order, int32_t num_layers,
                              int32_t d, const float* g_u, const float* g_i, const uint8_t* g_u_rows,
                              const uint8_t* g_i_rows, float* d_e0_u, float* d_e0_i, void* workspace,
                              size_t workspace_bytes, void* stream);
int cgx_propagate_bwd_frontier(const cgx_csr* by_user, const cgx_csr* by_item, int order, int32_t num_layers,
                               int32_t d, const float* g_u, const float* g_i, const uint8_t* g_u_rows,
                               const uint8_t* g_i_rows, const uint8_t* front_i, float* d_e0_u, float* d_e0_i,
                               void* workspace, size_t workspace_bytes, void* stream);
int cgx_batch_frontier(const cgx_csr* by_user, const int64_t* users, const int64_t* pos, const int64_t* neg,
                       int64_t batch, uint8_t* flags_i, uint8_t* flags_u, void* stream);

size_t cgx_bpr_plan_workspace_bytes(int64_t batch);
int cgx_bpr_plan(const int64_t* users, const int64_t* pos, const int64_t* neg, int64_t batch,
                 int32_t num_users, int32_t num_items, uint64_t* plan,
                 void* workspace, size_t workspace_bytes, void* stream);
size_t cgx_bpr_workspace_bytes(int64_t batch, int32_t num_users, int32_t num_items);
int cgx_bpr_fwd_bwd(const int64_t* users, const int64_t* pos, const int64_t* neg, int64_t batch,
                    int64_t batch_total, const uint64_t* plan, int32_t num_users, int32_t num_items, int32_t d,
                    const float* f_u, const float* f_i, const float* e0_u, const float* e0_i,
                    const float* pop, float reg_weight, float fair_weight,
                    float* loss_out, float* g_u, float* g_i,
                    int32_t* ego_rows, float* ego_coef,
                    void* workspace, size_t workspace_bytes, void* stream);
int cgx_bpr_apply_ego(const int32_t* ego_rows, const float* ego_coef, int64_t n_entries,
                      int32_t num_users, int32_t d, const float* e0_u, const float* e0_i,
                      float* d_e0_u, float* d_e0_i, void* stream);
int cgx_bpr_mark_rows(const int32_t* ego_rows, int64_t n_entries, int32_t num_users, uint8_t* nz_u, uint8_t* nz_i,
                      void* stream);
int cgx_bpr_clear_rows(const int32_t* ego_rows, int64_t n_entries, int32_t num_users, int32_t d, float* g_u,
                       float* g_i, uint8_t* nz_u, uint8_t* nz_i, void* stream);

size_t cgx_sampler_build_workspace_bytes(int32_t num_items);
int cgx_sampler_build(const int32_t* deg_i, int32_t num_items, double gamma,
                      int32_t* items_by_deg, int32_t* class_start, float* class_prob,
                      int32_t* class_alias, int32_t* n_classes,
                      void* workspace, size_t workspace_bytes, void* stream);

int cgx_sample_triples(const int64_t* users, int64_t batch, const int64_t* samp_indptr,
                       const int32_t* samp_idx, int32_t num_items,
                       const int32_t* items_by_deg, const int32_t* class_start,
                       const float* class_prob, const int32_t* class_alias, const int32_t* n_classes,
                       float mix_pop, int32_t max_tries, uint64_t seed, uint64_t offset,
                       const uint64_t* offset_dev, int64_t* pos_out, int64_t* neg_out, void* stream);

int cgx_tick(uint64_t* counter, void* stream);
int cgx_adam_step(float* p0, const float* g0, float* m0, float* v0, int64_t n0,
                  float* p1, const float* g1, float* m1, float* v1, int64_t n1,
                  float lr, float beta1, float beta2, float eps,
                  const uint64_t* step_dev, int64_t step_host, void* stream);

int cgx_comm_alloc(size_t bytes, void** base_out);
int cgx_comm_free(void* base);
int cgx_comm_ipc_handle(void* base, void* handle_out_64);
int cgx_comm_ipc_open(const void* handle_64, void** peer_base_out);
int cgx_comm_ipc_close(void* peer_base);
int cgx_comm_allreduce(int rank, int world, void* const* peer_bases, size_t in_off, size_t out_off,
                       size_t flag_off, int64_t n_floats, const uint64_t* epoch_dev, void* stream);
int cgx_comm_status(const void* base, size_t flag_off, int world, uint32_t* error_out);
int cgx_comm_allreduce_nvls(int rank, int world, void* const* peer_bases, void* mc_base, size_t in_off,
                            size_t out_off, size_t flag_off, int64_t n_floats, const uint64_t* epoch_dev, void* stream);
int cgx_comm_allgather(int rank, int world, void* const* peer_bases, const void* src, size_t dst_off,
                       size_t flag_off, int64_t bytes_per_rank, const uint64_t* epoch_dev, void* stream);

int cgx_spmm_set_push_peers(void* const* peer_bases, int world);
int cgx_spmm_push(const cgx_csr* m, int use_bwd_values, int32_t d, const float* X, const uint8_t* x_row_nonzero,
                  size_t stage_off, int rank, int world, int32_t rows_per,
                  void* workspace, size_t workspace_bytes, void* stream);
int cgx_comm_allreduce_pushed(int rank, int world, void* const* peer_bases, size_t stage_off, size_t out_off,
                              size_t flag_off, int64_t n_rows, int32_t d, int32_t rows_per,
                              const uint64_t* epoch_dev, void* stream);

int cgx_comm_timing(uint64_t* out4);

size_t cgx_eval_topk_workspace_bytes(int64_t n_users, int32_t num_items, int32_t d, int32_t k,
                                     int precision);
int cgx_eval_topk(const int64_t* users, int64_t n_users, const float* f_u, const float* f_i,
                  int32_t num_items, int32_t d, const int64_t* train_indptr, const int32_t* train_idx,
                  int32_t k, int precision, int32_t* out_ids, float* out_scores,
                  void* workspace, size_t workspace_bytes, void* stream);

int cgx_eval_topk_uses_tensor_cores(int32_t d, int32_t k, int precision);

int cgx_score_candidates(const int64_t* users, const int64_t* cand, int64_t n_users, int32_t n_cand,
                         int32_t d, const float* f_u, const float* f_i, float* scores, void* stream);

int cgx_eval_candidates(const int64_t* users, int64_t n_users, const int64_t* train_indptr,
                        const int32_t* train_idx, const int64_t* test_indptr, const int32_t* test_idx,
                        int32_t num_items, int32_t n_neg, uint64_t seed, int64_t* cand, void* stream);

int cgx_rank_candidates(const float* scores, const int64_t* cand, int64_t n_users, int32_t n_cand,
                        int64_t* ranked, void* stream);

size_t cgx_eval_metrics_workspace_bytes(int64_t n_users, int32_t n_ks);
int cgx_eval_metrics(const int32_t* ranked, int64_t n_users, int32_t ld, const int64_t* users,
                     const int64_t* test_indptr, const int32_t* test_idx, const int32_t* gt_single,
                     int32_t num_items, const int32_t* ks_host, int32_t n_ks, const int64_t* item_pop,
                     int64_t total_train, const uint8_t* group, uint32_t* bitmaps, double* out,
                     void* workspace, size_t workspace_bytes, void* stream);

int cgx_eval_coverage(const uint32_t* bitmaps, int32_t num_items, int32_t n_ks, uint64_t* counts, void* stream);

#ifdef __cplusplus
}
#endif
#if defined(__GNUC__)
#pragma GCC visibility pop
#endif
#endif
```

Baseline: 1.471 billion.

## Compact masked SpMM rows into a work list instead of early-exit masking

Replaces the per-item output-row mask check inside the SpMM kernel with a compacted work list built by a flag/scan/scatter pass, and launches a grid-stride kernel capped at a number of waves over only the selected items. The huge-row finish kernel likewise iterates only over listed chunks. This aims to avoid launching and scheduling threads for rows whose outputs are not needed, at the cost of three extra small kernels (flags, scan, scatter) per masked product. It also folds the memset of d_e0_i into the scale kernel by writing zeros for inactive rows.

After: 1.519 billion (median of 6 runs). +3.2%, better.

```diff
diff --git a/beyond-binary-fake-user-detection-a-credibility-aware-graph-based-recommender-system_b200/_lib.py b/beyond-binary-fake-user-detection-a-credibility-aware-graph-based-recommender-system_b200/_lib.py
--- a/beyond-binary-fake-user-detection-a-credibility-aware-graph-based-recommender-system_b200/_lib.py
+++ b/beyond-binary-fake-user-detection-a-credibility-aware-graph-based-recommender-system_b200/_lib.py
@@ -63,6 +63,9 @@
     "cgx_row_flags": (C.c_int, [_P, C.c_int64, C.c_int32, _P, _P]),
     "cgx_spmm_ex": (C.c_int, [_CSR, C.c_int, C.c_int32, _P, _P, _P, _P, _P, _P, C.c_float, _P, C.c_size_t, _P]),
     "cgx_spmm_set_l2_table_bytes": (C.c_int64, [C.c_int64]),
+    "cgx_work_list_bytes": (C.c_size_t, [_CSR]),
+    "cgx_work_list_workspace_bytes": (C.c_size_t, [_CSR]),
+    "cgx_work_list": (C.c_int, [_CSR, _P, _P, _P, C.c_size_t, _P]),
     "cgx_propagate_workspace_bytes": (C.c_size_t, [_CSR, _CSR, C.c_int32]),
     "cgx_propagate_workspace_bytes_for": (C.c_size_t, [_CSR, _CSR, C.c_int32, C.c_int]),
     "cgx_propagate_fwd": (C.c_int, [_CSR, _CSR, C.c_int, C.c_int32, C.c_int32, _P, _P, _P, _P, _P,
diff --git a/beyond-binary-fake-user-detection-a-credibility-aware-graph-based-recommender-system_b200/csrc/spmm.cu b/beyond-binary-fake-user-detection-a-credibility-aware-graph-based-recommender-system_b200/csrc/spmm.cu
--- a/beyond-binary-fake-user-detection-a-credibility-aware-graph-based-recommender-system_b200/csrc/spmm.cu
+++ b/beyond-binary-fake-user-detection-a-credibility-aware-graph-based-recommender-system_b200/csrc/spmm.cu
@@ -202,21 +202,16 @@
   int32_t n_chunks, n_huge;
 };
 
-template <int G, int V, int UNR, int MINB, bool NZ, bool PUSH, bool HOT>
-__global__ void __launch_bounds__(SP_THREADS, MINB) k_spmm(const int32_t* __restrict__ idx,
-                                                           const float* __restrict__ val, int64_t n_items,
-                                                           SpmmSched sc, const float4* __restrict__ X,
-                                                           float4* __restrict__ Y, const float4* ACC_IN,
-                                                           float4* ACC_OUT, float acc_scale, float4* partial,
-                                                           const uint8_t* __restrict__ nz,
-                                                           const uint8_t* __restrict__ acc_nz,
-                                                           const uint8_t* __restrict__ out_rows,
-                                                           const int4* __restrict__ work, const SpmmPush ps_in) {
-  const SpmmPush ps = PUSH ? ps_in : SpmmPush{0ull, 0, 0};
+template <int G, int V, int UNR, bool NZ, bool PUSH, bool HOT, bool LISTED>
+__device__ __forceinline__ void spmm_item(uint32_t listed, const int32_t* __restrict__ idx,
+                                          const float* __restrict__ val, int64_t n_items, const SpmmSched sc,
+                                          const float4* __restrict__ X, float4* __restrict__ Y,
+                                          const float4* ACC_IN, float4* ACC_OUT, float acc_scale, float4* partial,
+                                          const uint8_t* __restrict__ nz, const uint8_t* __restrict__ acc_nz,
+                                          const int4* __restrict__ work, const SpmmPush ps) {
   constexpr int ROW4 = G * V;
-  asm volatile("griddepcontrol.launch_dependents;");
   const int lane = threadIdx.x & (G - 1);
-  const uint32_t item = (blockIdx.x * uint32_t(SP_THREADS) + threadIdx.x) / G;
+  const uint32_t item = LISTED ? listed : (blockIdx.x * uint32_t(SP_THREADS) + threadIdx.x) / G;
   const unsigned mask = group_mask<G>();
   float4 acc[V];
 #pragma unroll
@@ -232,10 +227,7 @@
     cf = ld_idx<HOT>(idx + lane);
     wf = ld_val<HOT>(val + lane);
   }
-  asm volatile("griddepcontrol.wait;" ::: "memory");
-  if (NZ && !PUSH && out_rows != nullptr &&
-      __ldg(out_rows + (item >= sc.n_chunks ? wd.w : __ldg(sc.perm + wd.w))) == 0)
-    return;
+  if (!LISTED) asm volatile("griddepcontrol.wait;" ::: "memory");
   gather_batches<G, V, UNR, NZ, HOT>(idx, val, wd.z, X, lane, mask, cf, wf, acc, nz);
   if (item >= sc.n_chunks) {
     epilogue<G, V, HOT>(wd.w, lane, acc, Y, ACC_IN, ACC_OUT, acc_scale, acc_nz, ps);
@@ -263,17 +255,41 @@
   if (lane == 0) sc.arrive[k] = 0;
 }
 
+template <int G, int V, int UNR, int MINB, bool NZ, bool PUSH, bool HOT, bool LIST = false>
+__global__ void __launch_bounds__(SP_THREADS, MINB) k_spmm(const int32_t* __restrict__ idx,
+                                                           const float* __restrict__ val, int64_t n_items,
+                                                           SpmmSched sc, const float4* __restrict__ X,
+                                                           float4* __restrict__ Y, const float4* ACC_IN,
+                                                           float4* ACC_OUT, float acc_scale, float4* partial,
+                                                           const uint8_t* __restrict__ nz,
+                                                           const uint8_t* __restrict__ acc_nz,
+                                                           const uint32_t* __restrict__ list,
+                                                           const int4* __restrict__ work, const SpmmPush ps_in) {
+  const SpmmPush ps = PUSH ? ps_in : SpmmPush{0ull, 0, 0};
+  asm volatile("griddepcontrol.launch_dependents;");
+  if constexpr (!LIST) {
+    spmm_item<G, V, UNR, NZ, PUSH, HOT, false>(0, idx, val, n_items, sc, X, Y, ACC_IN, ACC_OUT, acc_scale, partial,
+                                               nz, acc_nz, work, ps);
+  } else {
+    asm volatile("griddepcontrol.wait;" ::: "memory");
+    const uint32_t n = __ldg(list), groups = gridDim.x * uint32_t(SP_THREADS / G);
+    for (uint32_t j = (blockIdx.x * uint32_t(SP_THREADS) + threadIdx.x) / G; j < n; j += groups)
+      spmm_item<G, V, UNR, NZ, PUSH, HOT, true>(__ldg(list + 1 + j), idx, val, n_items, sc, X, Y, ACC_IN, ACC_OUT,
+                                                acc_scale, partial, nz, acc_nz, work, ps);
+  }
+}
+
 template <int G, int V>
 __global__ void __launch_bounds__(SP_THREADS) k_spmm_finish(SpmmSched sc, const float4* __restrict__ partial,
                                                             float4* __restrict__ Y, const float4* ACC_IN,
                                                             float4* ACC_OUT, float acc_scale,
                                                             const uint8_t* __restrict__ acc_nz,
-                                                            const uint8_t* __restrict__ out_rows, const SpmmPush ps) {
+                                                            const uint32_t* __restrict__ huge, const SpmmPush ps) {
   constexpr int GROUPS = SP_THREADS / G;
   constexpr int ROW4 = G * V;
   __shared__ float4 red[GROUPS][ROW4];
-  const int k = blockIdx.x;
-  if (out_rows != nullptr && __ldg(out_rows + __ldg(sc.perm + k)) == 0) return;
+  if (huge != nullptr && blockIdx.x >= __ldg(huge)) return;
+  const int k = huge != nullptr ? int(__ldg(huge + 1 + blockIdx.x)) : int(blockIdx.x);
   const int lane = threadIdx.x & (G - 1), grp = threadIdx.x / G;
   const int c0 = __ldg(sc.chunk_ptr + k), c1 = __ldg(sc.chunk_ptr + k + 1);
   float4 acc[V];
@@ -318,12 +334,18 @@
   return CGX_OK;
 }
 
+static int64_t work_items(const cgx_csr* m) { return int64_t(m->n_chunks) + (m->n_rows - m->n_long); }
+
+constexpr int64_t LIST_WAVES = 64;
+template <int V, int UNR>
+constexpr int list_unr() { return V == 1 ? UNR / 2 : UNR; }
 template <int G, int V, int UNR, int MINB, bool NZ, bool PUSH, bool HOT>
 static int launch_spmm(const cgx_csr* m, const float* val, const float* X, float* Y, const float* ACC_IN,
                        float* ACC_OUT, float acc_scale, void* workspace, size_t workspace_bytes,
-                       cudaStream_t stream, const uint8_t* nz, const uint8_t* acc_nz, const uint8_t* out_rows,
+                       cudaStream_t stream, const uint8_t* nz, const uint8_t* acc_nz, const uint32_t* list,
                        const SpmmPush ps) {
   constexpr int GROUPS = SP_THREADS / G;
+  constexpr int LIST_UNR = list_unr<V, UNR>();
   float4* partial = nullptr;
   if (m->n_long > 0) {
     size_t need = size_t(m->n_chunks) * G * V * sizeof(float4);
@@ -332,7 +354,7 @@
     partial = static_cast<float4*>(workspace);
   }
   SpmmSched sc{m->perm, m->chunk_ptr, m->arrive, m->n_chunks, m->n_huge};
-  const int64_t items = int64_t(m->n_chunks) + (m->n_rows - m->n_long);
+  const int64_t items = work_items(m);
   cudaLaunchConfig_t cfg = {};
   cfg.gridDim = dim3((unsigned)ceil_div(items, GROUPS));
   cfg.blockDim = dim3(SP_THREADS);
@@ -343,30 +365,48 @@
   attr[0].val.programmaticStreamSerializationAllowed = option(CGX_OPT_PDL) != 0 ? 1 : 0;
   cfg.attrs = attr;
   cfg.numAttrs = 1;
-  CGX_CUDA(cudaLaunchKernelEx(&cfg, k_spmm<G, V, UNR, MINB, NZ, PUSH, HOT>, HOT ? m->idx_hint : m->idx, val, items, sc,
-                              reinterpret_cast<const float4*>(X), reinterpret_cast<float4*>(Y),
-                              reinterpret_cast<const float4*>(ACC_IN), reinterpret_cast<float4*>(ACC_OUT), acc_scale,
-                              partial, nz, acc_nz, out_rows, static_cast<const int4*>(m->work), ps));
+  const uint32_t* huge = nullptr;
+  if (list == nullptr) {
+    CGX_CUDA(cudaLaunchKernelEx(&cfg, k_spmm<G, V, UNR, MINB, NZ, PUSH, HOT>, HOT ? m->idx_hint : m->idx, val, items,
+                                sc, reinterpret_cast<const float4*>(X), reinterpret_cast<float4*>(Y),
+                                reinterpret_cast<const float4*>(ACC_IN), reinterpret_cast<float4*>(ACC_OUT),
+                                acc_scale, partial, nz, acc_nz, nullptr, static_cast<const int4*>(m->work), ps));
+  } else if constexpr (!PUSH && !HOT) {
+    auto kern = k_spmm<G, V, LIST_UNR, MINB, NZ, PUSH, HOT, true>;
+    int dev = 0, sms = 0, per_sm = 0;
+    CGX_CUDA(cudaGetDevice(&dev));
+    CGX_CUDA(cudaDeviceGetAttribute(&sms, cudaDevAttrMultiProcessorCount, dev));
+    CGX_CUDA(cudaOccupancyMaxActiveBlocksPerMultiprocessor(&per_sm, kern, SP_THREADS, 0));
+    const int64_t cap = LIST_WAVES * sms * (per_sm > 0 ? per_sm : 1);
+    if (cap < int64_t(cfg.gridDim.x)) cfg.gridDim = dim3((unsigned)cap);
+    CGX_CUDA(cudaLaunchKernelEx(&cfg, kern, m->idx, val, items, sc, reinterpret_cast<const float4*>(X),
+                                reinterpret_cast<float4*>(Y), reinterpret_cast<const float4*>(ACC_IN),
+                                reinterpret_cast<float4*>(ACC_OUT), acc_scale, partial, nz, acc_nz, list,
+                                static_cast<const int4*>(m->work), ps));
+    huge = list + 1 + items;
+  } else {
+    CGX_REQUIRE(false, CGX_ERR_ARG, "spmm: a work list needs a product without push mode or hints");
+  }
   CGX_LAUNCH_CHECK();
   if (m->n_huge > 0) {
     k_spmm_finish<G, V><<<(unsigned)m->n_huge, SP_THREADS, 0, stream>>>(
         sc, partial, reinterpret_cast<float4*>(Y), reinterpret_cast<const float4*>(ACC_IN),
-        reinterpret_cast<float4*>(ACC_OUT), acc_scale, acc_nz, out_rows, ps);
+        reinterpret_cast<float4*>(ACC_OUT), acc_scale, acc_nz, huge, ps);
     CGX_LAUNCH_CHECK();
   }
   return CGX_OK;
 }
 
-#define CGX_SPMM_ARGS m, val, X, Y, ACC_IN, ACC_OUT, acc_scale, ws, ws_bytes, stream, nz, acc_nz, out_rows, ps
+#define CGX_SPMM_ARGS m, val, X, Y, ACC_IN, ACC_OUT, acc_scale, ws, ws_bytes, stream, nz, acc_nz, list, ps
 
 template <int G, int V, int UNR>
 static int spmm_flavour(const cgx_csr* m, const float* val, const float* X, float* Y, const float* ACC_IN,
                         float* ACC_OUT, float acc_scale, void* ws, size_t ws_bytes, cudaStream_t stream,
-                        const uint8_t* nz, const uint8_t* acc_nz, const uint8_t* out_rows, const SpmmPush ps,
+                        const uint8_t* nz, const uint8_t* acc_nz, const uint32_t* list, const SpmmPush ps,
                         bool hot) {
   const bool push = ps.rows_per > 0;
   if constexpr (V == 2) {
-    if (hot && nz == nullptr) {
+    if (hot && nz == nullptr && list == nullptr) {
       if (push) return launch_spmm<G, V, UNR, 4, false, true, true>(CGX_SPMM_ARGS);
       return launch_spmm<G, V, UNR, 4, false, false, true>(CGX_SPMM_ARGS);
     }
@@ -379,18 +419,17 @@
   return launch_spmm<G, V, UNR, 4, false, false, false>(CGX_SPMM_ARGS);
 }
 
-#define CGX_FLAVOUR_ARGS m, val, X, Y, ACC_IN, ACC_OUT, acc_scale, ws, ws_bytes, stream, nz, acc_nz, out_rows, ps, hot
+#define CGX_FLAVOUR_ARGS m, val, X, Y, ACC_IN, ACC_OUT, acc_scale, ws, ws_bytes, stream, nz, acc_nz, list, ps, hot
 
 static int spmm_dispatch(const cgx_csr* m, int use_bwd, int32_t d, const float* X, float* Y, const float* ACC_IN,
                          float* ACC_OUT, float acc_scale, void* ws, size_t ws_bytes, cudaStream_t stream,
                          const uint8_t* nz = nullptr, const SpmmPush ps = SpmmPush{0ull, 0, 0},
-                         const uint8_t* acc_nz = nullptr, const uint8_t* out_rows = nullptr) {
+                         const uint8_t* acc_nz = nullptr, const uint32_t* list = nullptr) {
   CGX_REQUIRE(m && m->perm && m->work && (m->nnz == 0 || (m->idx && m->val_fwd && m->val_bwd)) && X, CGX_ERR_ARG,
               "spmm: NULL pointer (cgx_csr needs idx, both value arrays and the cgx_row_schedule* outputs)");
   CGX_REQUIRE(m->n_long == 0 || (m->chunk_ptr && m->arrive), CGX_ERR_ARG, "spmm: chunk tables missing");
   CGX_REQUIRE(Y || ACC_OUT || ps.rows_per > 0, CGX_ERR_ARG, "spmm: no output requested");
-  CGX_REQUIRE(out_rows == nullptr || (nz != nullptr && ps.rows_per == 0), CGX_ERR_ARG,
-              "spmm: an output-row mask needs gather flags and no push mode");
+  CGX_REQUIRE(list == nullptr || ps.rows_per == 0, CGX_ERR_ARG, "spmm: a work list needs a product without push mode");
   const float* val = use_bwd ? m->val_bwd : m->val_fwd;
   if (m->n_rows == 0) return CGX_OK;
   const bool beyond_l2 = int64_t(m->n_cols) * int64_t(d) * 4 > option(CGX_OPT_L2_TABLE_BYTES);
@@ -425,11 +464,77 @@
 
 static size_t spmm_ws(const cgx_csr* m, int32_t d) { return align_up(size_t(m ? m->n_chunks : 0) * d * 4); }
 
+struct ListSrc {
+  const int32_t* perm;
+  const int32_t* chunk_row;
+  int64_t n_items;
+  int32_t n_chunks, n_long;
+};
+__device__ __forceinline__ uint32_t list_flag(const ListSrc& s, int64_t j, const uint8_t* __restrict__ rows) {
+  const int64_t k = j < s.n_chunks ? int64_t(__ldg(s.chunk_row + j))
+                                   : (j < s.n_items ? j - s.n_chunks + s.n_long : j - s.n_items);
+  return __ldg(rows + __ldg(s.perm + k)) != 0 ? 1u : 0u;
+}
+__global__ void k_list_flags(ListSrc s, int64_t n, const uint8_t* __restrict__ rows, uint32_t* __restrict__ sel) {
+  const int64_t j = int64_t(blockIdx.x) * blockDim.x + threadIdx.x;
+  if (j < n) sel[j] = list_flag(s, j, rows);
+}
+__global__ void k_list_scatter(ListSrc s, int64_t n, const uint8_t* __restrict__ rows,
+                               const uint32_t* __restrict__ pos, uint32_t* __restrict__ list) {
+  const int64_t j = int64_t(blockIdx.x) * blockDim.x + threadIdx.x;
+  if (j >= n) return;
+  const uint32_t f = list_flag(s, j, rows), p = pos[j];
+  uint32_t* huge = list + 1 + s.n_items;
+  if (j < s.n_items) {
+    if (f) list[1 + p] = uint32_t(j);
+    if (j == s.n_items - 1) {
+      list[0] = p + f;
+      if (n == s.n_items) huge[0] = 0;
+    }
+  } else {
+    const uint32_t base = pos[s.n_items];
+    if (f) huge[1 + p - base] = uint32_t(j - s.n_items);
+    if (j == n - 1) huge[0] = p + f - base;
+  }
+}
+
+static int64_t list_entries(const cgx_csr* m) { return work_items(m) + m->n_huge; }
+static size_t list_bytes(const cgx_csr* m) { return align_up(size_t(list_entries(m) + 2) * 4); }
+static size_t list_ws_bytes(const cgx_csr* m) {
+  return align_up(size_t(list_entries(m)) * 4) + scan_temp_bytes(list_entries(m));
+}
+
+static int work_list(const cgx_csr* m, const uint8_t* rows, uint32_t* list, void* ws, size_t ws_bytes,
+                     cudaStream_t stream) {
+  CGX_REQUIRE(m && m->perm && rows && list && (m->n_long == 0 || m->chunk_row), CGX_ERR_ARG,
+              "work_list: NULL pointer");
+  CGX_REQUIRE(m->n_rows > 0, CGX_ERR_ARG, "work_list: empty row order");
+  CGX_REQUIRE(ws != nullptr && ws_bytes >= list_ws_bytes(m), CGX_ERR_WORKSPACE, "work_list: workspace too small");
+  const int64_t n = list_entries(m);
+  const ListSrc s{m->perm, m->chunk_row, work_items(m), m->n_chunks, m->n_long};
+  uint32_t* sel = static_cast<uint32_t*>(ws);
+  const size_t used = align_up(size_t(n) * 4);
+  k_list_flags<<<(unsigned)ceil_div(n, 256), 256, 0, stream>>>(s, n, rows, sel);
+  CGX_LAUNCH_CHECK();
+  CGX_TRY(exclusive_scan_u32(sel, sel, n, nullptr, static_cast<char*>(ws) + used, ws_bytes - used, stream));
+  k_list_scatter<<<(unsigned)ceil_div(n, 256), 256, 0, stream>>>(s, n, rows, sel, list);
+  CGX_LAUNCH_CHECK();
+  return CGX_OK;
+}
+
 }
 
 using namespace cgx;
 
 extern "C" size_t cgx_spmm_workspace_bytes(const cgx_csr* m, int32_t d) { return spmm_ws(m, d); }
+
+extern "C" size_t cgx_work_list_bytes(const cgx_csr* m) { return m ? list_bytes(m) : 0; }
+extern "C" size_t cgx_work_list_workspace_bytes(const cgx_csr* m) { return m ? list_ws_bytes(m) : 0; }
+
+extern "C" int cgx_work_list(const cgx_csr* m, const uint8_t* rows, uint32_t* list, void* workspace,
+                             size_t workspace_bytes, void* stream) {
+  return work_list(m, rows, list, workspace, workspace_bytes, static_cast<cudaStream_t>(stream));
+}
 
 extern "C" int cgx_spmm(const cgx_csr* m, int use_bwd_values, int32_t d, const float* X, float* Y,
                         const float* ACC_IN, float* ACC_OUT, float acc_scale, void* workspace,
@@ -541,11 +646,27 @@
   return CGX_OK;
 }
 
+static size_t max_size(size_t a, size_t b) { return a > b ? a : b; }
 static size_t propagate_ws(const cgx_csr* by_user, const cgx_csr* by_item, int32_t d, int n_buf) {
   if (!by_user || !by_item) return 0;
-  size_t long_ws = spmm_ws(by_user, d) > spmm_ws(by_item, d) ? spmm_ws(by_user, d) : spmm_ws(by_item, d);
+  size_t long_ws = max_size(spmm_ws(by_user, d), spmm_ws(by_item, d));
   return n_buf * (align_up(size_t(by_user->n_rows) * d * 4) + align_up(size_t(by_item->n_rows) * d * 4)) + long_ws +
-         align_up(size_t(by_user->n_rows)) + align_up(size_t(by_item->n_rows)) + 256;
+         align_up(size_t(by_user->n_rows)) + align_up(size_t(by_item->n_rows)) +
+         max_size(list_bytes(by_user), list_bytes(by_item)) + max_size(list_ws_bytes(by_user), list_ws_bytes(by_item)) +
+         256;
+}
+
+struct ListWs {
+  uint32_t* list;
+  void* ws;
+  size_t ws_bytes;
+};
+static ListWs take_list(Arena& ws, const cgx_csr* by_user, const cgx_csr* by_item) {
+  ListWs l;
+  l.list = ws.take<uint32_t>(max_size(list_bytes(by_user), list_bytes(by_item)) / 4);
+  l.ws_bytes = max_size(list_ws_bytes(by_user), list_ws_bytes(by_item));
+  l.ws = ws.take<char>(l.ws_bytes);
+  return l;
 }
 
 extern "C" size_t cgx_propagate_workspace_bytes(const cgx_csr* by_user, const cgx_csr* by_item, int32_t d) {
@@ -574,8 +695,6 @@
   CGX_REQUIRE(K >= 1, CGX_ERR_ARG, "propagate_fwd: num_layers must be >= 1");
   CGX_REQUIRE(0 <= layer_begin && layer_begin <= layer_end && layer_end <= K, CGX_ERR_ARG,
               "propagate_fwd: layers [%d, %d) outside [0, %d)", layer_begin, layer_end, K);
-  CGX_REQUIRE((rows_u == nullptr && rows_i == nullptr) || all_rows != nullptr, CGX_ERR_ARG,
-              "propagate_fwd: output-row masks need all_rows");
   CGX_REQUIRE(order == CGX_ORDER_JACOBI || order == CGX_ORDER_GS, CGX_ERR_ARG, "propagate_fwd: bad order");
   CGX_REQUIRE(by_user->n_rows == by_item->n_cols && by_user->n_cols == by_item->n_rows, CGX_ERR_ARG,
               "propagate_fwd: operator shapes disagree");
@@ -592,6 +711,7 @@
   ib[1] = one ? ib[0] : ws.take<float>(I * d);
   size_t lws = spmm_ws(by_user, d) > spmm_ws(by_item, d) ? spmm_ws(by_user, d) : spmm_ws(by_item, d);
   void* lw = ws.take<char>(lws);
+  const ListWs lst = take_list(ws, by_user, by_item);
   CGX_REQUIRE(ws.ok, CGX_ERR_WORKSPACE, "propagate_fwd: workspace too small");
   const float s = 1.0f / float(K + 1);
   const SpmmPush nops{0ull, 0, 0};
@@ -605,11 +725,13 @@
     const uint8_t* mu = last ? rows_u : nullptr;
     const uint8_t* mi = last ? rows_i : nullptr;
     const bool need_ni = !last || order == CGX_ORDER_GS;
+    if (mi) CGX_TRY(work_list(by_item, mi, lst.list, lst.ws, lst.ws_bytes, stream));
     CGX_TRY(spmm_dispatch(by_item, 0, d, cu, need_ni ? ni : nullptr, first ? e0_i : out_i, out_i, sc, lw, lws,
-                          stream, mi ? all_rows : nullptr, nops, nullptr, mi));
+                          stream, nullptr, nops, nullptr, mi ? lst.list : nullptr));
     const float* src = order == CGX_ORDER_JACOBI ? ci : ni;
+    if (mu) CGX_TRY(work_list(by_user, mu, lst.list, lst.ws, lst.ws_bytes, stream));
     CGX_TRY(spmm_dispatch(by_user, 0, d, src, last ? nullptr : nu, first ? e0_u : out_u, out_u, sc, lw, lws,
-                          stream, mu ? all_rows : nullptr, nops, nullptr, mu));
+                          stream, nullptr, nops, nullptr, mu ? lst.list : nullptr));
   }
   return CGX_OK;
 }
@@ -617,8 +739,10 @@
 __global__ void k_scale_rows(const float4* __restrict__ in, const uint8_t* __restrict__ nz, float4* __restrict__ out,
                              int64_t n_rows, int32_t row4, float s) {
   const int64_t r = (int64_t(blockIdx.x) * blockDim.x + threadIdx.x) / 32;
-  if (r >= n_rows || __ldg(nz + r) == 0) return;
-  for (int p = threadIdx.x & 31; p < row4; p += 32) out[r * row4 + p] = scale4(in[r * row4 + p], s);
+  if (r >= n_rows) return;
+  const bool on = __ldg(nz + r) != 0;
+  for (int p = threadIdx.x & 31; p < row4; p += 32)
+    out[r * row4 + p] = on ? scale4(in[r * row4 + p], s) : make_float4(0.f, 0.f, 0.f, 0.f);
 }
 
 extern "C" int cgx_propagate_bwd(const cgx_csr* by_user, const cgx_csr* by_item, int order, int32_t K, int32_t d,
@@ -665,6 +789,7 @@
   const bool sparse = given || option(CGX_OPT_SPARSE_FIRST_ADJOINT) != 0;
   uint8_t* nz_u = given ? const_cast<uint8_t*>(g_u_rows) : ws.take<uint8_t>(U);
   uint8_t* nz_i = given ? const_cast<uint8_t*>(g_i_rows) : ws.take<uint8_t>(I);
+  const ListWs lst = take_list(ws, by_user, by_item);
   CGX_REQUIRE(ws.ok, CGX_ERR_WORKSPACE, "propagate_bwd: workspace too small");
   const uint8_t* front = sparse ? front_i : nullptr;
   if (order == CGX_ORDER_JACOBI) {
@@ -684,8 +809,10 @@
       const uint8_t* bi_nz = sp ? nz_i : (k == 1 ? front : nullptr);
       CGX_TRY(spmm_dispatch(by_user, 1, d, bi, nullptr, g_u, nu, sc, lw, lws, stream, bi_nz, nops,
                             sparse ? nz_u : nullptr));
+      const bool masked = front != nullptr && k == 0 && !last;
+      if (masked) CGX_TRY(work_list(by_item, front, lst.list, lst.ws, lst.ws_bytes, stream));
       CGX_TRY(spmm_dispatch(by_item, 1, d, bu, nullptr, g_i, ni, sc, lw, lws, stream, sp ? nz_u : nullptr, nops,
-                            sparse ? nz_i : nullptr, k == 0 && !last ? front : nullptr));
+                            sparse ? nz_i : nullptr, masked ? lst.list : nullptr));
       bu = nu;
       bi = ni;
     }
@@ -701,15 +828,16 @@
       float* ni = ib[0];
       float* nu = last ? d_e0_u : ub[k & 1];
       const uint8_t* f0 = k == 0 ? front : nullptr;
+      if (f0) CGX_TRY(work_list(by_item, f0, lst.list, lst.ws, lst.ws_bytes, stream));
       CGX_TRY(spmm_dispatch(by_item, 1, d, bu, nullptr, g_i, ni, 1.0f, lw, lws, stream,
-                            sparse && k == 0 ? nz_u : nullptr, nops, sparse ? nz_i : nullptr, f0));
+                            sparse && k == 0 ? nz_u : nullptr, nops, sparse ? nz_i : nullptr,
+                            f0 ? lst.list : nullptr));
       CGX_TRY(spmm_dispatch(by_user, 1, d, ni, nullptr, g_u, nu, last ? s : 1.0f, lw, lws, stream, f0, nops,
                             sparse ? nz_u : nullptr));
       bu = nu;
     }
     const int64_t n4 = I * d / 4;
     if (given) {
-      CGX_CUDA(cudaMemsetAsync(d_e0_i, 0, size_t(I) * d * 4, stream));
       if (I > 0) {
         k_scale_rows<<<(unsigned)ceil_div(I * 32, 256), 256, 0, stream>>>(
             reinterpret_cast<const float4*>(g_i), nz_i, reinterpret_cast<float4*>(d_e0_i), I, d / 4, s);
diff --git a/beyond-binary-fake-user-detection-a-credibility-aware-graph-based-recommender-system_b200/model.py b/beyond-binary-fake-user-detection-a-credibility-aware-graph-based-recommender-system_b200/model.py
--- a/beyond-binary-fake-user-detection-a-credibility-aware-graph-based-recommender-system_b200/model.py
+++ b/beyond-binary-fake-user-detection-a-credibility-aware-graph-based-recommender-system_b200/model.py
@@ -351,7 +351,7 @@
         self._bufs = {}
         self._graph = None
         self._defer_final = None
-        self._fws = self._all_rows = None
+        self._fws = None
         self._pending = False
         self._final_error = None
 
@@ -389,7 +389,7 @@
             try:
                 check(lib().cgx_propagate_fwd_layers(g.by_user.ref(), g.by_item.ref(), order, K, d, ptr(eu), ptr(ei),
                                                      ptr(self._f_u), ptr(self._f_i), K - 1, K, ptr(rest_u),
-                                                     ptr(rest_i), ptr(self._all_rows), ptr(self._fws),
+                                                     ptr(rest_i), None, ptr(self._fws),
                                                      self._fws.numel(), stream_ptr(dev)))
             except _lib.CgxError as e:
                 self._final_error = e
@@ -423,7 +423,6 @@
         if defer and self._fws is None:
             self._fws = workspace(lib().cgx_propagate_workspace_bytes_for(g.by_user.ref(), g.by_item.ref(), d, order),
                                   dev)
-            self._all_rows = torch.ones(max(g.num_users, g.num_items), dtype=torch.uint8, device=dev)
         front = self.front_i if beyond_l2 or defer else None
         marks = []
         self._pending, self._final_error = False, None
@@ -444,7 +443,7 @@
                 main.wait_stream(self.side)
                 check(lib().cgx_propagate_fwd_layers(g.by_user.ref(), g.by_item.ref(), order, K, d, ptr(eu), ptr(ei),
                                                      ptr(self._f_u), ptr(self._f_i), K - 1, K, ptr(self.batch_u),
-                                                     ptr(self.front_i), ptr(self._all_rows), ptr(fws), fws.numel(),
+                                                     ptr(self.front_i), None, ptr(fws), fws.numel(),
                                                      st))
                 self._mark(marks)
                 self._pending = True
diff --git a/include/credgcn.h b/include/credgcn.h
--- a/include/credgcn.h
+++ b/include/credgcn.h
@@ -112,6 +112,11 @@
                 float* Y, const float* ACC_IN, const uint8_t* acc_row_nonzero, float* ACC_OUT, float acc_scale,
                 void* workspace, size_t workspace_bytes, void* stream);
 
+size_t cgx_work_list_bytes(const cgx_csr* m);
+size_t cgx_work_list_workspace_bytes(const cgx_csr* m);
+int cgx_work_list(const cgx_csr* m, const uint8_t* rows, uint32_t* list, void* workspace, size_t workspace_bytes,
+                  void* stream);
+
 int64_t cgx_spmm_set_l2_table_bytes(int64_t bytes);
 
 size_t cgx_propagate_workspace_bytes(const cgx_csr* by_user, const cgx_csr* by_item, int32_t d);
```
